# BBillot/SynthSR

Hardware: AMD Instinct MI355X
Metric: training volumes/sec (160^3 fp32, 5-level U-Net) (higher is better)
Workload: dtype f32; 1 GPU; configs[1]: brain_generator 160^3 batch=1 (training() defaults) + 5-level 3-D U-Net (24..384 features, Cin=2) fwd/bwd + Adam, fp32, random-init; global_batch=1, parallelism=dp1, conv_arithmetic=split

## Files before the change

include/synthsr_hip_tuning.h:

```cpp
#ifndef SYNTHSR_HIP_TUNING_H
#define SYNTHSR_HIP_TUNING_H
#ifdef __cplusplus
extern "C" {
#endif

int synthsr_split_tile_schedule(int kernel, int ntiles, int ny, int block_x, int block_yz, int out[4]);

int synthsr_set_deterministic(int on);
int synthsr_set_deterministic_workspace(void* planes, unsigned long long bytes);
unsigned long long synthsr_deterministic_workspace_demand(void);
int synthsr_deterministic_status(void);

#ifdef __cplusplus
}
#endif
#endif
```

synthsr_amd/_lib.py:

```python
import ctypes
import os
from ctypes import POINTER, Structure, c_char_p, c_double, c_float, c_int, c_int32, c_int64, c_uint32, c_uint64, c_void_p

_HERE = os.path.dirname(os.path.abspath(__file__))
LIB_PATH = os.environ.get('SYNTHSR_HIP_LIB') or os.path.join(_HERE, 'libsynthsr_hip.so')

_lib = None

I3 = c_int * 3
F12 = c_float * 12


class DeformParams(Structure):
    _fields_ = [('in_shape', c_int * 3), ('out_shape', c_int * 3), ('crop', c_int * 3), ('flip', c_int),
                ('has_field', c_int), ('has_affine', c_int), ('half_shape', c_int * 3), ('aff', c_float * 12),
                ('n_channels', c_int), ('lut_size', c_int), ('swap_lut_size', c_int), ('bias_on', c_int * 4),
                ('bias_shape', (c_int * 3) * 4), ('clip_hi', c_float), ('use_philox', c_int),
                ('philox_key', c_uint32 * 2), ('philox_offset', c_uint64), ('chan_first', c_int), ('n_channels_total', c_int),
                ('label_bytes', c_int)]


class ConvCtx(Structure):
    _fields_ = [('arithmetic', c_int), ('reserved0', c_int), ('workspace', c_void_p), ('workspace_bytes', c_uint64),
                ('reserved', c_int * 2)]


_P = c_void_p
_S = c_void_p
_C = POINTER(ConvCtx)

SIGNATURES = {
    'synthsr_abi_version': (c_int, []),
    'synthsr_build_arch': (c_char_p, []),
    'synthsr_resize_f32': (c_int, [_P, _P, c_int, POINTER(c_int), POINTER(c_int), c_int, _S]),
    'synthsr_svf_integrate': (c_int, [_P, _P, POINTER(c_int), c_int, _S]),
    'synthsr_affine_resample_linear': (c_int, [_P, _P, c_int, POINTER(c_int), POINTER(c_float), _S]),
    'synthsr_deform_gmm': (c_int, [_P, _P, _P, _P, _P, _P, _P, _P, _P, POINTER(DeformParams), _S]),
    'synthsr_mimic_acquisition': (c_int, [_P, _P, POINTER(c_int), POINTER(c_int), POINTER(c_float), POINTER(c_float),
                                          POINTER(c_float), c_int, c_int, c_int, _S]),
    'synthsr_deform_gmm_real': (c_int, [_P, _P, _P, _P, _P, _P, _P, _P, _P, _P, _P, _P, POINTER(DeformParams), _S]),
    'synthsr_minmax_init': (c_int, [_P, c_int, _S]),
    'synthsr_minmax_reduce': (c_int, [_P, c_int64, _P, _S]),
    'synthsr_normalise_gamma': (c_int, [_P, _P, c_int64, _P, c_float, _S]),
    'synthsr_blur3d': (c_int, [_P, _P, POINTER(c_int), _P, POINTER(c_int), c_int, c_int, c_int, c_float, _S]),
    'synthsr_normalise_blur2': (c_int, [_P, POINTER(c_int), _P, c_float, _P, _P, _P, _P, c_int, c_int, c_int, c_float, _S]),
    'synthsr_outer3': (c_int, [_P, _P, POINTER(c_int), c_int, c_int, _S]),
    'synthsr_copy_strided': (c_int, [_P, _P, c_int64, c_int, c_int, c_int, c_int, _S]),
    'synthsr_conv3d_pack': (c_int64, [_C, _P, _P, POINTER(c_int), c_int, c_int, c_int, _S]),
    'synthsr_conv3d_fwd': (c_int, [_C, _P, _P, _P, _P, POINTER(c_int), c_int, c_int, c_int, _S]),
    'synthsr_conv3d_fwd_stats': (c_int, [_C, _P, _P, _P, _P, POINTER(c_int), c_int, c_int, c_int, _P, _P, _S]),
    'synthsr_bn_stats_from_partials': (c_int, [_P, c_int, c_int64, c_int, _P, _S]),
    'synthsr_conv3d_fwd_add': (c_int, [_C, _P, _P, _P, _P, _P, POINTER(c_int), c_int, c_int, c_int, _S]),
    'synthsr_split_tile_schedule': (c_int, [c_int, c_int, c_int, c_int, c_int, POINTER(c_int)]),
    'synthsr_conv3d_wgrad_runs_split': (c_int, [_C, POINTER(c_int), c_int, c_int]),
    'synthsr_set_deterministic': (c_int, [c_int]),
    'synthsr_set_deterministic_workspace': (c_int, [_P, c_uint64]),
    'synthsr_deterministic_workspace_demand': (c_uint64, []),
    'synthsr_conv_workspace_bytes': (c_uint64, []),
    'synthsr_deterministic_status': (c_int, []),
    'synthsr_conv3d_plan': (c_int, [_C, POINTER(c_int), c_int, c_int, c_int, POINTER(c_int64)]),
    'synthsr_conv3d_pack_all': (c_int, [_P, _P, _P, c_int, _S]),
    'synthsr_conv3d_pack_ex': (c_int64, [_C, _P, _P, POINTER(c_int), c_int, c_int, c_int, c_int, c_int, c_int, _S]),
    'synthsr_conv3d_up_fwd': (c_int, [_C, _P, _P, _P, _P, _P, POINTER(c_int), c_int, c_int, c_int, _S]),
    'synthsr_conv3d_up_dgrad': (c_int, [_C, _P, _P, _P, POINTER(c_int), c_int, c_int, _S]),
    'synthsr_conv3d_up_wgrad': (c_int, [_C, _P, _P, _P, POINTER(c_int), c_int, c_int, _S]),
    'synthsr_conv3d_up_wgrad_runs_split': (c_int, [_C, POINTER(c_int), c_int, c_int]),
    'synthsr_conv3d_up_unpack': (c_int, [_P, _P, c_int, c_int, c_int, c_int, _S]),
    'synthsr_conv3d_wgrad_bias': (c_int, [_C, _P, _P, _P, _P, POINTER(c_int), c_int, c_int, c_int, c_int, _S]),
    'synthsr_conv3d_wgrad_ex': (c_int, [_C, _P, _P, _P, POINTER(c_int), c_int, c_int, c_int, c_int, _S]),
    'synthsr_conv3d_wgrad': (c_int, [_C, _P, _P, _P, POINTER(c_int), c_int, c_int, _S]),
    'synthsr_head_loss_fwd_ab': (c_int, [_P, POINTER(c_int), c_int, _P, _P, _P, c_float, _P, _P, _P, c_int, c_int, _P, _P, _P, _P, c_int, POINTER(c_int), _P, _S]),
    'synthsr_head_bwd_from_sums': (c_int, [_P, c_int, _P, _P, _P, _P, _P, _P, _S]),
    'synthsr_head_loss_fwd_bf16': (c_int, [_P, POINTER(c_int), c_int, _P, _P, _P, c_float, _P, _P, c_int, _P, c_int, POINTER(c_int), _P, _P, _P, _P, c_int, POINTER(c_int), _S]),
    'synthsr_conv3d_bf16_pack': (c_int64, [_P, _P, c_int, c_int, c_int, c_int, c_int, _S]),
    'synthsr_conv3d_bf16_pack_ex': (c_int64, [_P, _P, c_int, c_int, c_int, c_int, c_int, c_int, _S]),
    'synthsr_conv3d_bf16_pack_job': (c_int, [c_int, c_int, c_int, c_int, c_int, c_int, _P]),
    'synthsr_conv3d_bf16_wgrad_part': (c_int, [_P, _P, _P, _P, POINTER(c_int), c_int, c_int, c_int, c_int, _S]),
    'synthsr_conv3d_bf16_up_fwd': (c_int, [_P, _P, _P, POINTER(c_int), c_int, c_int, _S]),
    'synthsr_conv3d_bf16_up_dgrad': (c_int, [_P, _P, _P, POINTER(c_int), c_int, c_int, _P, c_int64, _S]),
    'synthsr_conv3d_bf16_up_wgrad': (c_int, [_P, _P, _P, POINTER(c_int), c_int, c_int, _S]),
    'synthsr_conv3d_bf16_pack_all': (c_int, [_P, _P, _P, c_int, _S]),
    'synthsr_conv3d_bf16_fwd': (c_int, [_P, _P, _P, _P, POINTER(c_int), c_int, c_int, c_int, _P, _P, _P, c_int64, _S]),
    'synthsr_conv3d_bf16_fwd_ex': (c_int, [_P, _P, _P, _P, POINTER(c_int), c_int, c_int, c_int, c_float, _P, _P, _P, c_int64, _S]),
    'synthsr_bf16_subsample_odd': (c_int, [_P, _P, _P, POINTER(c_int), c_int, c_float, _S]),
    'synthsr_bf16_zero_insert_odd': (c_int, [_P, _P, POINTER(c_int), c_int, _S]),
    'synthsr_conv3d_bf16_stats_scratch': (c_int64, [POINTER(c_int), c_int, c_int]),
    'synthsr_conv3d_bf16_wgrad': (c_int, [_P, _P, _P, _P, POINTER(c_int), c_int, c_int, c_int, c_int, _S]),
    'synthsr_f32_to_bf16_pad': (c_int, [_P, _P, c_int64, c_int, c_int, _S]),
    'synthsr_elu_bwd': (c_int, [_P, _P, _P, _P, _P, c_int64, c_int, _S]),
    'synthsr_scale_channels': (c_int, [_P, _P, c_int64, c_int, _P, c_int64, _S]),
    'synthsr_elu_bwd_drop': (c_int, [_P, _P, _P, _P, _P, c_int64, c_int, _P, _P, c_float, _P, _P, _P, _P, c_int64, _S]),
    'synthsr_bn_elu_bwd': (c_int, [_P, _P, _P, _P, _P, c_int64, c_int, _P, _P, c_float, _P, _S]),
    'synthsr_bn_stats': (c_int, [_P, c_int64, c_int, _P, _P, _S]),
    'synthsr_bn_apply': (c_int, [_P, _P, c_int64, c_int, _P, _P, _P, c_float, _S]),
    'synthsr_bn_maxpool': (c_int, [_P, _P, POINTER(c_int), c_int, _P, _P, _P, c_float, _S]),
    'synthsr_bn_maxpool_bwd': (c_int, [_P, _P, _P, POINTER(c_int), c_int, _P, _P, _P, c_float, _S]),
    'synthsr_bn_maxpool_bwd_ex': (c_int, [_P, _P, _P, POINTER(c_int), c_int, _P, _P, _P, c_float, _P, _S]),
    'synthsr_bn_pool_elu_bwd': (c_int, [_P, _P, _P, _P, _P, POINTER(c_int), c_int, _P, _P, _P, _P, c_float, _S]),
    'synthsr_act_bwd': (c_int, [_P, _P, _P, _P, _P, c_int64, c_int, c_int, _S]),
    'synthsr_bn_act_bwd': (c_int, [_P, _P, _P, _P, _P, c_int64, c_int, _P, _P, c_float, _P, c_int, _S]),
    'synthsr_bn_act_bwd_head': (c_int, [_P, _P, _P, _P, _P, c_int64, c_int, _P, _P, c_float, _P, c_int, _S]),
    'synthsr_act_bwd_drop': (c_int, [_P, _P, _P, _P, _P, c_int64, c_int, _P, _P, c_float, _P, _P, _P, _P, c_int64, c_int, _S]),
    'synthsr_bn_pool_act_bwd': (c_int, [_P, _P, _P, _P, _P, POINTER(c_int), c_int, _P, _P, _P, _P, c_float, c_int, _S]),
    'synthsr_bn_bwd_reduce': (c_int, [_P, _P, c_int64, c_int, _P, c_float, _P, _S]),
    'synthsr_bn_bwd_apply': (c_int, [_P, _P, _P, c_int64, c_int, _P, _P, c_float, _P, _S]),
    'synthsr_upsample_concat': (c_int, [_P, _P, _P, POINTER(c_int), c_int, c_int, _P, _P, _P, c_float, _S]),
    'synthsr_upsample_concat_bwd': (c_int, [_P, _P, _P, POINTER(c_int), c_int, c_int, _S]),
    'synthsr_head_l1_fwd': (c_int, [_P, c_int64, c_int, _P, _P, _P, c_float, _P, _P, _P, c_int, c_int, _P, _P, _P,
                                    _P, _S]),
    'synthsr_head_loss_fwd': (c_int, [_P, _P, c_int, _P, _P, _P, c_float, _P, _P, c_int, _P, c_int, _P, _P, _P, _P,
                                      _P, c_int, _P, _S]),
    'synthsr_head_bwd_multi': (c_int, [_P, _P, c_int64, c_int, c_int, _P, _P, _P, c_float, _P, _P, _P, _P, _S]),
    'synthsr_ssim_products': (c_int, [_P, _P, _P, _P, _P, _S]),
    'synthsr_ssim_filter': (c_int, [_P, _P, _P, c_int, c_int, c_int, _P, _S]),
    'synthsr_ssim_point': (c_int, [_P, c_int64, c_float, c_float, _P, _P, _S]),
    'synthsr_ssim_combine': (c_int, [_P, _P, _P, _P, _P, _P, _S]),
    'synthsr_conv3d_stride_unpack': (c_int, [_P, _P, c_int, c_int, _S]),
    'synthsr_bias_leaky_relu': (c_int, [_P, _P, _P, c_int64, c_int, c_float, _S]),
    'synthsr_colsum': (c_int, [_P, c_int64, c_int, _P, _S]),
    'synthsr_mul': (c_int, [_P, _P, _P, c_int64, _S]),
    'synthsr_lut_gather': (c_int, [_P, _P, c_int, _P, c_int64, _S]),
    'synthsr_leaky_relu': (c_int, [_P, _P, _P, c_int64, c_float, _S]),
    'synthsr_dense_fwd': (c_int, [_P, _P, _P, _P, c_int64, c_int, _S]),
    'synthsr_dense_bwd': (c_int, [_P, _P, _P, _P, _P, c_int64, c_int, _S]),
    'synthsr_axpby': (c_int, [_P, _P, _P, c_int64, c_float, c_float, _S]),
    'synthsr_sumsq': (c_int, [_P, c_int64, _P, _S]),
    'synthsr_bn_elu_bwd_head': (c_int, [_P, _P, _P, _P, _P, c_int64, c_int, _P, _P, c_float, _P, _S]),
    'synthsr_head_bwd_ex': (c_int, [_P, _P, c_int64, c_int, _P, _P, _P, c_float, _P, _P, _P, _P, _P, _S]),
    'synthsr_seg_head_fwd': (c_int, [_P, c_int64, c_int, _P, _P, _P, c_float, _P, _P, c_int, _P, _S]),
    'synthsr_seg_dice_sums': (c_int, [_P, _P, c_int64, c_int, _P, _P, c_int, _P, _S]),
    'synthsr_seg_dice_bwd': (c_int, [_P, _P, c_int64, c_int, c_int, _P, _P, _P, c_int, _P, c_float, _P, _S]),
    'synthsr_seg_head_dice_fwd': (c_int, [_P, c_int64, c_int, _P, _P, _P, c_float, _P, _P, c_int, _P, _P, c_int, _P, _P, _S]),
    'synthsr_seg_head_dice_bwd': (c_int, [_P, _P, _P, c_int, _P, c_int64, c_int, c_int, _P, _P, _P, c_float, _P, _P, c_float, _P,
                                          _P, _P, _S]),
    'synthsr_seg_head_argmax': (c_int, [_P, c_int64, c_int, _P, _P, _P, c_float, _P, _P, c_int, _P, _P, _S]),
    'synthsr_seg_head_tta_argmax': (c_int, [_P, POINTER(c_int), c_int, _P, _P, _P, c_float, _P, _P, c_int, _P, _P, _P, _P, _P,
                                            _S]),
    'synthsr_seg_label_counts': (c_int, [_P, _P, c_int64, _P, c_int, c_int, _P, _S]),
    'synthsr_head_bwd': (c_int, [_P, _P, c_int64, c_int, _P, _P, _P, c_float, _P, _P, _P, _P, _S]),
    'synthsr_adam_step': (c_int, [_P, _P, _P, _P, c_int64, c_float, c_float, c_float, c_float, c_float, _S]),
}

for _name in ('synthsr_elu_bwd', 'synthsr_bn_elu_bwd', 'synthsr_bn_elu_bwd_head', 'synthsr_elu_bwd_drop', 'synthsr_bn_pool_elu_bwd',
              'synthsr_act_bwd', 'synthsr_bn_act_bwd', 'synthsr_bn_act_bwd_head', 'synthsr_act_bwd_drop', 'synthsr_bn_pool_act_bwd',
              'synthsr_scale_channels', 'synthsr_bn_stats', 'synthsr_bn_apply', 'synthsr_bn_maxpool', 'synthsr_bn_maxpool_bwd',
              'synthsr_bn_maxpool_bwd_ex', 'synthsr_bn_bwd_reduce', 'synthsr_upsample_concat', 'synthsr_upsample_concat_bwd',
              'synthsr_head_loss_fwd_ab', 'synthsr_head_bwd_multi', 'synthsr_head_bwd_ex', 'synthsr_head_bwd'):
    SIGNATURES[_name + '_bf16'] = SIGNATURES[_name]


CONV_ARITHMETICS = ('fp32_mfma', 'split', 'split9')


class SynthSRHipError(RuntimeError):
    pass


def load():
    global _lib
    if _lib is not None:
        return _lib
    if not os.path.exists(LIB_PATH):
        raise SynthSRHipError('%s not found: build it with `python -m synthsr_amd.build` (hipcc, gfx950). '
                              'There is no CPU fallback.' % LIB_PATH)
    lib = ctypes.CDLL(LIB_PATH)
    for name, (res, args) in SIGNATURES.items():
        fn = getattr(lib, name)
        fn.restype = res
        fn.argtypes = args
    _lib = lib
    return lib


def check(rc, what='', planes=False):
    if rc == 0:
        return
    if rc == -1:
        raise ValueError('synthsr_hip: invalid argument / unsupported shape in %s' % what)
    if rc == -3 and planes:
        raise SynthSRHipError('synthsr_hip: %s needs more deterministic weight-gradient planes than the registered plane buffer '
                              'holds, even after registering a larger one (include/synthsr_hip_tuning.h: '
                              'synthsr_set_deterministic_workspace)' % what)
    if rc == -3:
        raise SynthSRHipError('synthsr_hip: %s needs scratch and the conv context carries no (or too small a) workspace '
                              '(include/synthsr_hip.h: synthsr_conv_ctx.workspace)' % what)
    raise SynthSRHipError('synthsr_hip: HIP launch error (%d) in %s' % (rc, what))


def i3(seq):
    return I3(*[int(s) for s in seq])


def ptr(t):
    if t is None:
        return None
    assert t.is_cuda and t.is_contiguous(), 'tensors handed to the HIP library must be contiguous device tensors'
    return c_void_p(t.data_ptr())


def stream():
    import torch
    return c_void_p(torch.cuda.current_stream().cuda_stream)
```

synthsr_amd/csrc/common.h:

```cpp
#pragma once
#include <hip/hip_runtime.h>
#include <stdint.h>
#include <type_traits>
#include "../../include/synthsr_hip.h"

#define SYN_CHECK_LAUNCH()                                 \
  do {                                                     \
    hipError_t e__ = hipGetLastError();                    \
    if (e__ != hipSuccess) return SYNTHSR_ELAUNCH;         \
  } while (0)

static inline int64_t syn_cdiv(int64_t a, int64_t b) { return (a + b - 1) / b; }

static inline int syn_grid(int64_t n, int block, int max_blocks = 256 * 16) {
  int64_t g = syn_cdiv(n, block);
  if (g > max_blocks) g = max_blocks;
  if (g < 1) g = 1;
  return (int)g;
}

#ifdef __HIPCC__
__device__ static inline void syn_block_range(int64_t n, int64_t& lo, int64_t& hi) {
  const int G = (int)gridDim.x, b = (int)blockIdx.x;
  const int pos = (G % 8 == 0) ? (b & 7) * (G >> 3) + (b >> 3) : b;
// ... 87 lines not shown
    }
    __syncthreads();
    if (tid < n) {
      double t = 0.0;
      for (int p = 0; p < P; ++p) t += s_col[p * n + tid];
      part[tid] = (float)t;
    }
  } else {
    for (int i = tid; i < n; i += nt) {
      double t = 0.0;
      for (int w = 0; w < nwg; ++w) t += (double)__builtin_nontemporal_load(d->scratch + (size_t)w * n + i);
      part[i] = (float)t;
    }
  }
  if (syn_tid0()) d->arrivals = 0;
  __syncthreads();
  return true;
}

__device__ __forceinline__ void syn_det_gather_end(int n) {
  SynDet* d = g_syn_det;
  if (d && (long long)syn_wg_count() * n > d->scratch_floats)
    syn_turn_end(&d->chain[SYN_DET_CHAINS - 1], syn_wg_linear(), syn_wg_count());
}

#include <atomic>
struct SynOncePerDevice {
  std::atomic<uint64_t> bits{0};
  bool needed() const {
    int dev = -1;
    if (hipGetDevice(&dev) != hipSuccess || dev < 0 || dev > 63) return true;
    return !(bits.load(std::memory_order_acquire) & (1ull << dev));
  }
  void done() {
    int dev = -1;
    if (hipGetDevice(&dev) == hipSuccess && dev >= 0 && dev <= 63) bits.fetch_or(1ull << dev, std::memory_order_release);
  }
  struct Guard {
    SynOncePerDevice* o;
    bool need;
    ~Guard() { if (need) o->done(); }
    explicit operator bool() const { return need; }
  };
  Guard first() { return Guard{this, needed()}; }
};
template <auto Kern>
void max_dyn_smem(size_t bytes) {
  static SynOncePerDevice done;
  if (auto once_ = done.first()) {
    (void)hipFuncSetAttribute(reinterpret_cast<const void*>(Kern), hipFuncAttributeMaxDynamicSharedMemorySize, (int)bytes);
  }
}
template <auto Kern, auto KernR, class... Args>
void launch_smem(bool relu, dim3 grid, dim3 block, size_t smem, hipStream_t st, Args... args) {
  if (relu) {
    max_dyn_smem<KernR>(smem);
    hipLaunchKernelGGL(KernR, grid, block, smem, st, args...);
  } else {
    max_dyn_smem<Kern>(smem);
    hipLaunchKernelGGL(Kern, grid, block, smem, st, args...);
  }
}

struct DetRun {
  float* planes = nullptr;
  float* dw = nullptr;
  float* dbias = nullptr;
  int64_t dw_elems = 0, stride = 0;
  int cout = 0, gx = 0;
};
extern "C" int syn_det_enabled();
extern "C" int syn_det_prepare(DetRun* d, float** dw, float** dbias, int64_t dw_elems, int cout, int gx, hipStream_t st);
extern "C" int syn_det_finish(const DetRun* d, hipStream_t st);

#define SYN_DET_SETTER(name)                                                                              \
  extern "C" __attribute__((visibility("hidden"))) int syn_det_set_##name(SynDet* p) {                   \
    return hipMemcpyToSymbol(HIP_SYMBOL(g_syn_det), &p, sizeof(p)) == hipSuccess ? 0 : 1;                 \
  }
#endif

__host__ __device__ static inline int syn_up_axis_taps(int p, int s, int t[2]) {
  if (p == 0) {
    if (s == 0) { t[0] = 0; return 1; }
    if (s == 1) { t[0] = 1; t[1] = 2; return 2; }
    return 0;
  }
  if (s == 1) { t[0] = 0; t[1] = 1; return 2; }
  if (s == 2) { t[0] = 2; return 1; }
  return 0;
}

__host__ __device__ static inline uint32_t syn_f2ord(float f) {
  union { float f; uint32_t u; } c;
  c.f = f;
  return (c.u & 0x80000000u) ? ~c.u : (c.u | 0x80000000u);
}
__host__ __device__ static inline float syn_ord2f(uint32_t u) {
  union { float f; uint32_t u; } c;
  c.u = (u & 0x80000000u) ? (u & 0x7fffffffu) : ~u;
  return c.f;
}

#ifdef __HIPCC__
__device__ __forceinline__ void syn_minmax_update(uint32_t* mm, float mn, float mx) {
  const uint32_t lo = syn_f2ord(mn), hi = syn_f2ord(mx);
  if (lo < __hip_atomic_load(&mm[0], __ATOMIC_RELAXED, __HIP_MEMORY_SCOPE_AGENT)) atomicMin(&mm[0], lo);
  if (hi > __hip_atomic_load(&mm[1], __ATOMIC_RELAXED, __HIP_MEMORY_SCOPE_AGENT)) atomicMax(&mm[1], hi);
}
#endif

#ifdef __HIPCC__
__device__ __forceinline__ uint32_t syn_pack_bf16x2(float lo, float hi) {
  typedef __bf16 syn_bf16x2 __attribute__((ext_vector_type(2)));
  const syn_bf16x2 v = {(__bf16)lo, (__bf16)hi};
  return __builtin_bit_cast(uint32_t, v);
}
__device__ __forceinline__ void syn_split3(float f0, float f1, uint32_t& p0, uint32_t& p1, uint32_t& p2) {
  p0 = syn_pack_bf16x2(f0, f1);
  float r0 = f0 - __uint_as_float(p0 << 16), r1 = f1 - __uint_as_float(p0 & 0xffff0000u);
  p1 = syn_pack_bf16x2(r0, r1);
  r0 -= __uint_as_float(p1 << 16);
  r1 -= __uint_as_float(p1 & 0xffff0000u);
  p2 = syn_pack_bf16x2(r0, r1);
}
#endif

#ifdef __HIPCC__
template <int I, int N, class F>
__device__ __forceinline__ void sfor(F&& f) {
  if constexpr (I < N) {
    f(std::integral_constant<int, I>{});
    sfor<I + 1, N>(f);
  }
}

__device__ __forceinline__ float elu_f(float v) {
  const float e = __builtin_amdgcn_exp2f(v * 1.44269504088896341f) - 1.f;
  const float p = v * fmaf(v, fmaf(v, fmaf(v, fmaf(v, 1.f / 120.f, 1.f / 24.f), 1.f / 6.f), 0.5f), 1.f);
  const float n = v > -0.125f ? p : e;
  return v > 0.f ? v : n;
}
__device__ __forceinline__ float elu_dy(float y) { return y > 0.f ? 1.f : y + 1.f; }
template <bool RELU>
__device__ __forceinline__ float act_f(float v) {
  if constexpr (RELU) return fmaxf(v, 0.f);
  else return elu_f(v);
}
template <bool RELU>
__device__ __forceinline__ float act_dy(float y) {
  if constexpr (RELU) return y > 0.f ? 1.f : 0.f;
  else return elu_dy(y);
}

constexpr int TZ = 4, TY = 4, TX = 16, HZ = TZ + 2, HY = TY + 2, HX = TX + 2, HVOX = HZ * HY * HX;
constexpr int SLAB_Z = 4;
__device__ __forceinline__ void tile_decode(int p, int tiles0, int tiles1, int tiles2, int& z0, int& y0, int& x0) {
  const int t12 = tiles1 * tiles2;
  const int s = p / (SLAB_Z * t12), r = p - s * SLAB_Z * t12;
  const int sz = min(SLAB_Z, tiles0 - s * SLAB_Z);
  const int t1 = r / (sz * tiles2), rr = r - t1 * sz * tiles2;
  const int zz = rr / tiles2, t2 = rr - zz * tiles2;
  z0 = (s * SLAB_Z + zz) * TZ;
  y0 = t1 * TY;
  x0 = t2 * TX;
}
#endif
static inline int syn_tile_grid_x(int slots, int ntiles) {
  int gx = slots / 8 * 8;
  if (gx < 8) gx = 8;
  while (gx > 8 && gx - 8 >= ntiles) gx -= 8;
  if (ntiles < 8) gx = ntiles;
  return gx;
}

__host__ __device__ inline bool syn_split_replanned(int vox_tiles, int co_tiles, int mt) {
  if (mt != 2 || co_tiles <= 3 || (co_tiles % 3) != 0 || (co_tiles % 2) != 0) return false;
  const long long u3 = (long long)vox_tiles * (co_tiles / 3);
  return u3 > 512 && u3 < 768;
}
__host__ __device__ inline int syn_split_plan_mt(int vox_tiles, int co_tiles, bool replan) {
  const int mt = co_tiles <= 3 ? co_tiles : ((co_tiles % 3) == 0 ? 3 : ((co_tiles % 2) == 0 ? 2 : 1));
  if (replan && mt == 3 && syn_split_replanned(vox_tiles, co_tiles, 2)) return 2;
  return mt;
}

__host__ __device__ constexpr int syn_split_tap(int slot) {
  const int p = slot >> 1, h = slot & 1;
  if (p < 9) return p * 3 + 2 * h;
  const int i = 2 * (p - 9) + h;
  return i < 9 ? i * 3 + 1 : -1;
}
__host__ __device__ constexpr int syn_split_tap8(int slot) {
  const int p = slot >> 1, h = slot & 1;
  return 4 * (p & 1) + 2 * h + (p >> 1);
}
__host__ __device__ constexpr int syn_split_voxel(int m) { return m < 4 ? 2 * m : (m >= 12 ? 2 * m - 16 : 2 * m - 7); }

__device__ static inline float syn_wave_sum(float v) {
#pragma unroll
  for (int o = 32; o > 0; o >>= 1) v += __shfl_xor(v, o, 64);
  return v;
}
__device__ static inline float syn_wave_min(float v) {
#pragma unroll
  for (int o = 32; o > 0; o >>= 1) v = fminf(v, __shfl_xor(v, o, 64));
  return v;
}
__device__ static inline float syn_wave_max(float v) {
#pragma unroll
  for (int o = 32; o > 0; o >>= 1) v = fmaxf(v, __shfl_xor(v, o, 64));
  return v;
}
```

synthsr_amd/csrc/conv3d.hip:

```cpp
#include "common.h"
#include <algorithm>
#include <cstddef>

SYN_DET_SETTER(conv3d)

namespace {

typedef float f32x4 __attribute__((ext_vector_type(4)));

constexpr int MAX_NT = 6;

__host__ __device__ inline int cdiv(int a, int b) { return (a + b - 1) / b; }

inline int ck_for(int Cin) { return (Cin % 24 == 0) ? 24 : 8; }
inline int ck_for_fwd(int Cin) { return (Cin % 24 == 0) ? 24 : ((Cin % 32 == 0) ? 32 : 8); }

typedef unsigned int u32x4 __attribute__((ext_vector_type(4)));
typedef unsigned int u32x2 __attribute__((ext_vector_type(2)));
__device__ __forceinline__ float4 ld4(const float* p) { return *reinterpret_cast<const float4*>(p); }

__device__ __forceinline__ int up_axis_taps(int p, int s, int t[2]) {
  if (p == 0) {
    if (s == 0) { t[0] = 0; return 1; }
    if (s == 1) { t[0] = 1; t[1] = 2; return 2; }
// ... 2462 lines not shown
      if (i < NJ - 1 || tid + 256 * i < PLANE4) {
#pragma unroll
        for (int hz = 0; hz < FH0; ++hz)
          *reinterpret_cast<float4*>(&lds[ldsa[i] + hz * (FH1 * FH2 * CKP)]) = stg[hz * NJ + i];
      }
    }
    __syncthreads();
    const bool has_next = t + G < ntiles;
    if (has_next) load_halo(t + G);
    int nz0 = z0, ny0 = y0, nx0 = x0;
    if (has_next) tile_origin(t + G, nz0, ny0, nx0);
    for (int z = 0; z < FT0; ++z) {
      float ar[8][3];
#pragma unroll
      for (int o = 0; o < 8; ++o)
#pragma unroll
        for (int r = 0; r < 3; ++r) ar[o][r] = an[o][r];
      if (z + 1 < FT0) {
        load_dz(z0, y0, x0, z + 1, an);
      } else if (has_next) {
        load_dz(nz0, ny0, nx0, 0, an);
      }
      int rb[NQ];
#pragma unroll
      for (int q = 0; q < NQ; ++q) rb[q] = rowoff[q] + z * (FH1 * FH2 * CKP);
      float xq[2][NQ];
#pragma unroll
      for (int q = 0; q < NQ; ++q) xq[0][q] = lds[rb[q]];
      sfor<0, 64>([&](auto S) {
        constexpr int sv = decltype(S)::value, o = sv / 8, k = sv % 8;
        constexpr int sn = sv + 1 < 64 ? sv + 1 : sv, on = sn / 8, kn = sn % 8;
        constexpr int nbase = ((on >> 1) * FH2 + 8 * (on & 1) + kn) * CKP;
#pragma unroll
        for (int q = 0; q < NQ; ++q) xq[(sv + 1) & 1][q] = lds[rb[q] + nbase];
        __builtin_amdgcn_sched_barrier(0);
        sfor<0, 6>([&](auto GI) {
          constexpr int g = decltype(GI)::value, GG = k * 6 + g;
#pragma unroll
          for (int q = 0; q < NQ; ++q)
            acc[q][g] = __builtin_amdgcn_mfma_f32_4x4x1f32(ar[o][GG / 16], xq[sv & 1][q], acc[q][g], 4, GG % 16, 0);
        });
        __builtin_amdgcn_sched_barrier(0);
      });
    }
    z0 = nz0;
    y0 = ny0;
    x0 = nx0;
  }
  dwc += (size_t)blockIdx.x * det_stride;
  for (int w = 0; w < 4; ++w) {
    __syncthreads();
    if (wave == w) {
#pragma unroll
      for (int q = 0; q < NQ; ++q) {
        const int blk = 16 * q + (lane >> 2);
        float* d = lds + (blk * 4 + (lane & 3)) * Cout;
#pragma unroll
        for (int g = 0; g < 6; ++g)
          *reinterpret_cast<float4*>(d + 4 * g) = make_float4(acc[q][g][0], acc[q][g][1], acc[q][g][2], acc[q][g][3]);
      }
    }
    __syncthreads();
    const int wp = (blockIdx.y & 1) * 4 + w, wz = (wp >> 2) & 1, wy = (wp >> 1) & 1, wx = wp & 1;
    float* dst = dwc + (size_t)wp * dwstride;
    for (int e = tid; e < 8 * CK * Cout; e += 256) {
      const int ti = e / (CK * Cout), r = e - ti * (CK * Cout);
      const int tap = ((wz + ((ti >> 2) & 1)) * 3 + (wy + ((ti >> 1) & 1))) * 3 + (wx + (ti & 1));
      atomicAdd(dst + ((size_t)tap * Cin + cc * CK) * Cout + r, lds[e]);
    }
  }
}

__global__ __launch_bounds__(256) void colsum_kernel(const float* __restrict__ x, int64_t n, int C,
                                                     float* __restrict__ out) {
  __shared__ float part[256];
  const int rows = C <= 256 ? 256 / C : 1;
  int* turn = nullptr;
  for (int c0 = 0; c0 < C; c0 += 256) {
    const int width = min(256, C - c0);
    const int r = threadIdx.x / width, c = threadIdx.x - r * width;
    float acc = 0.f;
    if (r < rows)
      for (int64_t v = (int64_t)blockIdx.x * rows + r; v < n; v += (int64_t)gridDim.x * rows) acc += x[v * C + c0 + c];
    part[threadIdx.x] = acc;
    __syncthreads();
    if (c0 == 0) turn = syn_turn_begin(0, blockIdx.x);
    if (threadIdx.x < width) {
      float t = 0.f;
      for (int k = 0; k < rows; ++k) t += part[k * width + threadIdx.x];
      atomicAdd(out + c0 + threadIdx.x, t);
    }
    __syncthreads();
  }
  syn_turn_end(turn, blockIdx.x, gridDim.x);
}

constexpr int SYN_MAX_DEVICES = 64;
struct SynDeviceState {
  int det = 0;
  SynDet* det_state = nullptr;
  float* det_planes = nullptr;
  size_t det_planes_floats = 0;
  unsigned long long det_demand_bytes = 0;
};
static SynDeviceState g_dev[SYN_MAX_DEVICES];
static SynDeviceState g_dev_invalid;
static SynDeviceState& dev_state() {
  int d = -1;
  if (hipGetDevice(&d) != hipSuccess || d < 0 || d >= SYN_MAX_DEVICES) return g_dev_invalid;
  return g_dev[d];
}
static inline int det_on() { return dev_state().det; }

constexpr int PLAN_KS_TARGET = 1024;
constexpr int PLAN_SPLIT_MIN_WGS = 200;

struct ConvCfg {
  int arith;
  int split;
  int nprod;
  void* ws;
  size_t ws_bytes;
};
static thread_local ConvCfg t_cfg = {1, 1, 6, nullptr, 0};
static inline const ConvCfg& cfg() { return t_cfg; }
struct CtxScope {
  ConvCfg prev;
  bool ok;
  explicit CtxScope(const synthsr_conv_ctx* ctx) : prev(t_cfg), ok(true) {
    const int a = ctx ? ctx->arithmetic : SYNTHSR_ARITH_SPLIT;
    if (a < 0 || a > 2 || (ctx && (ctx->reserved0 || ctx->reserved[0] || ctx->reserved[1] || (ctx->workspace_bytes && !ctx->workspace)))) {
      ok = false;
      return;
    }
    t_cfg = ConvCfg{a, a ? 1 : 0, a == 2 ? 9 : 6, ctx ? ctx->workspace : nullptr, ctx ? (size_t)ctx->workspace_bytes : 0};
  }
  ~CtxScope() { t_cfg = prev; }
};
constexpr size_t SYN_WORKSPACE_BOUND = (size_t)16 << 20;
static float* ctx_scratch(size_t bytes) {
  static_assert((size_t)2048 * 1536 * sizeof(float) <= SYN_WORKSPACE_BOUND, "first-layer weight-gradient partials");
  return (bytes <= SYN_WORKSPACE_BOUND && bytes <= cfg().ws_bytes) ? static_cast<float*>(cfg().ws) : nullptr;
}

extern "C" int syn_split_wgrad(const float* in, const float* dout, float* dw, float* dbias, const int s[3], int cin_total,
                               int ci_off, int Cin, int Cout, int nprod, hipStream_t st);
extern "C" int syn_split_upwgrad(const float* lo, const float* dout, float* dwc, const int s[3], int Cin, int Cout, int nprod,
                                 hipStream_t st);
extern "C" int syn_split_upfwd(const float* lo, const float* wp, const float* bias, const float* addend, float* out,
                               const int s[3], int Cin, int Cout, int mt, int act, int nprod, hipStream_t st);
extern "C" int syn_split_fwd_halves(const int s[3], int Cin, int nchunks, int stacked, int nprod);
extern "C" int syn_split_fwd(const float* in, const float* wp, const float* bias, const float* addend, float* out,
                             const int s[3], int Cin, int Cout, int mt, int nchunks, int act, float* stats, float* partial,
                             int upm, int stacked, int nprod, hipStream_t st);

inline bool wgrad_takes_split(const int s[3], int Cin, int Cout) {
  const int64_t vox = (int64_t)s[0] * s[1] * s[2];
  return cfg().split && (Cin % 8) == 0 && (Cout % 24) == 0 && vox * Cin * 4 < (1ll << 31) && vox * Cout * 4 < (1ll << 31);
}

inline bool up_wgrad_takes_split(const int s[3], int Cl, int Cout) {
  const int64_t vox = (int64_t)s[0] * s[1] * s[2];
  return cfg().split && cfg().nprod == 6 && (Cl % 16) == 0 && (Cout % 24) == 0 && vox * Cl * 4 < (1ll << 31) &&
         8 * vox * Cout * 4 < (1ll << 31);
}

struct FwdPlan {
  int nt, mt, ksplit, nchunks, ncc, ck, persist, p4, c2, brick, wn, wm, split, stacked;
  int pack_nt() const { return stacked ? -400 : split == 3 ? -300 - mt : (split == 2 ? -200 - mt : (split ? -100 - mt : (c2 ? -c2 : (p4 ? 0 : nt)))); }
  int64_t count() const {
    if (stacked) return (int64_t)ncc * 7 * 5 * 64 * 4;
    if (split) return (int64_t)3 * nchunks * ncc * (split >= 2 ? 2 : 7) * mt * 64 * 4;
    if (c2) return (int64_t)((27 * c2 * 6 + 15) / 16) * 64;
    if (p4) return (int64_t)ncc * 27 * 9 * 64;
    return (int64_t)nchunks * ncc * 27 * (ck / 8) * nt * 128;
  }
};

inline FwdPlan plan_fwd(const int s[3], int Cin, int Cout, int kind = 1) {
  const bool plain = kind == 1;
  FwdPlan p;
  p.split = 0;
  p.stacked = 0;
  if (cfg().split && (Cin % 8) == 0 && (Cout % 8) == 0) {
    const int64_t vox = (int64_t)s[0] * s[1] * s[2];
    const int ntiles = cdiv(Cout, 16);
    const int mt = syn_split_plan_mt(cdiv(s[0], 4) * cdiv(s[1], 4) * cdiv(s[2], 16), ntiles, kind != 2);
    const int nchunks = cdiv(ntiles, mt);
    const int64_t wgs = (int64_t)cdiv(s[0], 4) * cdiv(s[1], 4) * cdiv(s[2], 16) * nchunks;
    if (wgs >= PLAN_SPLIT_MIN_WGS && (kind == 0 ? 8 : 1) * vox * Cin * 4 < (1ll << 31) && (kind == 2 ? 8 : 1) * vox * Cout * 4 < (1ll << 31) &&
        (kind != 2 || nchunks == 1)) {
      p.split = plain ? 1 : (kind == 0 ? 2 : 3);
      p.ck = 8;
      p.ncc = Cin / 8;
      p.mt = mt;
      p.nt = mt;
      p.nchunks = nchunks;
      p.ksplit = 1;
      p.stacked = (plain && Cout == 24 && cfg().arith == 1) ? 1 : 0;
      p.persist = p.p4 = p.c2 = p.brick = 0;
      p.wn = p.wm = 1;
      return p;
    }
  }
  p.ck = ck_for_fwd(Cin);
  p.ncc = cdiv(Cin, p.ck);
  const int ntiles = cdiv(Cout, 16);
  auto wgs = [&](int mt, int nt) { return (int64_t)cdiv(s[0], FT0) * cdiv(s[1], mt) * cdiv(s[2], FT2) * cdiv(ntiles, nt); };
  p.mt = 4;
  int max_nt = MAX_NT;
  if (wgs(4, std::min(MAX_NT, ntiles)) < 768 || p.ck == 32) {
    p.mt = 2;
    max_nt = 3;
  }
  p.nchunks = cdiv(ntiles, max_nt);
  p.nt = cdiv(ntiles, p.nchunks);
  p.ksplit = 1;
  const bool lt2g = (int64_t)s[0] * s[1] * s[2] * Cin * 4 < (1ll << 31);
  p.persist = (p.mt == 4 && p.ck == 24 && p.nt <= 3 && (Cout % 4) == 0 && lt2g) ? 1 : 0;
  p.p4 = (p.persist && (kind == 1 || kind == 2) && Cout == 24 && (Cin % 24) == 0) ? 1 : 0;
  p.c2 = (plain && Cout == 24 && Cin <= 2 && lt2g) ? Cin : 0;
  p.brick = 0;
  p.wn = 1;
  p.wm = 1;
  if (p.ck == 24 && p.mt == 2 && lt2g && (Cout % 16) == 0 && (s[0] % 4) == 0 && (s[1] % 4) == 0 && (s[2] % 4) == 0 &&
      (s[2] % 16) != 0) {
    p.brick = 1;
    p.nt = (ntiles % 3 == 0) ? 3 : ((ntiles % 2 == 0) ? 2 : 1);
    p.nchunks = ntiles / p.nt;
    p.wn = (p.nchunks % 4 == 0) ? 4 : ((p.nchunks % 2 == 0) ? 2 : 1);
    p.wm = (p.wn <= 2 && (s[1] % 8) == 0) ? 2 : 1;
    if (p.wn == 1) {
      p.brick = 0;
      p.wm = 1;
      p.nchunks = cdiv(ntiles, max_nt);
      p.nt = cdiv(ntiles, p.nchunks);
    }
  }
  if (p.brick) {
    const int64_t w = (int64_t)(s[0] / 4) * (s[1] / (4 * p.wm)) * (s[2] / 4) * (p.nchunks / p.wn);
    p.ksplit = 1;
    if (w < 400 && p.ncc >= 2 && plain) {
      int ks = (int)cdiv(PLAN_KS_TARGET, (int)w);
      if (ks > p.ncc) ks = p.ncc;
      if (ks > 16) ks = 16;
      if (ks >= 2 && !det_on()) p.ksplit = ks;
    }
    return p;
  }
  const int64_t w = wgs(p.mt, p.nt);
  if (w < 512 && p.ncc >= 4 && plain) {
    int ks = (int)cdiv(PLAN_KS_TARGET, (int)w);
    if (ks > p.ncc / 2) ks = p.ncc / 2;
    if (ks > 8) ks = 8;
    if (ks >= 2 && !det_on()) p.ksplit = ks;
  }
  return p;
}

inline int parity_split(int64_t workgroups, const float* bias, int act, const ConvExt& ext) {
  if (det_on() || bias != nullptr || act != 0 || ext.addend != nullptr) return 1;
  int ps = 1;
  while (ps < 8 && workgroups * ps < 400) ps *= 2;
  return ps;
}

inline bool launch_act(int& act) {
  const bool relu = act >= 3;
  if (relu) act -= 2;
  return relu;
}

inline int splitk_begin(float* out, int64_t nout, int act, const ConvExt& ext, hipStream_t st) {
  if (ext.mode != 0) return SYNTHSR_EINVAL;
  if (act != 2 && ext.addend && ext.addend != out) return SYNTHSR_EINVAL;
  if ((act == 2 || !ext.addend) && hipMemsetAsync(out, 0, (size_t)nout * sizeof(float), st) != hipSuccess) return SYNTHSR_ELAUNCH;
  return SYNTHSR_OK;
}
inline int splitk_end(float* out, const float* bias, int64_t nout, int Cout, int act, bool relu, const ConvExt& ext,
                      hipStream_t st) {
  if (bias == nullptr && act == 0) return SYNTHSR_OK;
  hipLaunchKernelGGL((relu ? bias_act_kernel<true> : bias_act_kernel<false>), dim3(syn_grid(nout, 256)), dim3(256), 0, st, out,
                     bias, nout, Cout, act, act == 2 ? ext.addend : nullptr);
  return hipGetLastError() == hipSuccess ? SYNTHSR_OK : SYNTHSR_ELAUNCH;
}

template <int CK, int NT, int MT, bool KS>
int launch_fwd(const float* in, const float* wp, const float* bias, float* out, const int s[3], int Cin, int Cout,
               const FwdPlan& pl, int act, hipStream_t st, const ConvExt& ext) {
  const bool relu = launch_act(act);
  const int tiles0 = cdiv(s[0], FT0), tiles1 = cdiv(s[1], MT), tiles2 = cdiv(s[2], FT2);
  const size_t smem = (size_t)FH0 * (MT + 2) * FH2 * (CK + 4) * sizeof(float);
  const int64_t nout = (int64_t)s[0] * s[1] * s[2] * Cout;
  enum { GENERIC, LEAN27, LEAN8 } kern = GENERIC;
  if constexpr (CK == 24 && NT <= 3) {
    const int64_t in_bytes = (int64_t)s[0] * s[1] * s[2] * (ext.mode == 2 ? 8 : 1) * Cin * 4;
    const int64_t w_bytes = pl.count() * 4 * (ext.mode ? 8 : 1);
    if (in_bytes < (1ll << 31) && w_bytes < (1ll << 31)) kern = ext.mode == 0 ? LEAN27 : LEAN8;
  }
  if (KS) {
    if (const int rc = splitk_begin(out, nout, act, ext, st)) return rc;
  }
  int gz = KS ? pl.ksplit : (ext.mode == 1 ? 8 : 1);
  if (!KS && kern == LEAN8 && ext.mode == 2) {
    gz = parity_split((int64_t)tiles0 * tiles1 * tiles2 * pl.nchunks, bias, act, ext);
    if (gz > 1 && hipMemsetAsync(out, 0, (size_t)nout * sizeof(float), st) != hipSuccess) return SYNTHSR_ELAUNCH;
  }
// ... 517 lines not shown
      return syn_det_finish(&det, st);
    }
  }
  if constexpr (NTAPS == 27) {
    if (Cin <= 2 && Cout == 24 && (int64_t)shape[0] * shape[1] * shape[2] * Cout * 4 < (1ll << 31))
      return launch_wgrad_c2(in, dout, dw, ext.dbias, shape, Cin, st, ext);
    if (wgrad_takes_split(shape, Cin, Cout)) {
      const int rc = syn_split_wgrad(in, dout, dw, ext.dbias, shape, ext.cin_total, ext.ci_off, Cin, Cout, cfg().nprod, st);
      if (rc != SYNTHSR_EINVAL) return rc;
    }
  }
  if constexpr (NTAPS == 27) {
    const int64_t vox = (int64_t)shape[0] * shape[1] * shape[2];
    if (Cout == 24 && (Cin % 24) == 0 && vox * Cin * 4 < (1ll << 31) && vox * Cout * 4 < (1ll << 31)) {
      const int tiles0 = cdiv(shape[0], FT0), tiles1 = cdiv(shape[1], 4), tiles2 = cdiv(shape[2], FT2);
      const int ntiles = tiles0 * tiles1 * tiles2, ncc = Cin / 24;
      const size_t smem = (size_t)FH0 * 6 * FH2 * 28 * sizeof(float);
      max_dyn_smem<conv3d_wgrad_p4_kernel>(smem);
      int gx = std::max(8, ((512 / ncc) / 8) * 8);
      while (gx > 8 && gx > ntiles) gx -= 8;
      DetRun det;
      float* dbias = ext.dbias;
      if (const int rc_ = syn_det_prepare(&det, &dw, &dbias, (int64_t)27 * ext.cin_total * Cout, Cout, gx, st)) return rc_;
      hipLaunchKernelGGL(conv3d_wgrad_p4_kernel, dim3(gx, ncc), dim3(256), smem, st, in, dout, dw, shape[0], shape[1],
                         shape[2], Cin, tiles1, tiles2, ntiles, ext.cin_total, ext.ci_off, dbias, det.stride);
      if (hipGetLastError() != hipSuccess) return SYNTHSR_ELAUNCH;
      return syn_det_finish(&det, st);
    }
  }
  const int CK = ck_for(Cin);
  const int nt_all = cdiv(Cout, 16);
  const int nco = cdiv(nt_all, 3);
  const int NT = cdiv(nt_all, nco);
  if (CK == 24) {
    if (NT == 1) return launch_wgrad<24, 1, 1, NTAPS>(in, dout, dw, shape, Cin, Cout, st, ext);
    if (NT == 2) return launch_wgrad<24, 2, 1, NTAPS>(in, dout, dw, shape, Cin, Cout, st, ext);
    if constexpr (NTAPS == 27) return launch_wgrad<24, 3, 2, 27>(in, dout, dw, shape, Cin, Cout, st, ext);
    return launch_wgrad<24, 3, 1, NTAPS>(in, dout, dw, shape, Cin, Cout, st, ext);
  }
  if (NT == 1) return launch_wgrad<8, 1, 1, NTAPS>(in, dout, dw, shape, Cin, Cout, st, ext);
  if (NT == 2) return launch_wgrad<8, 2, 1, NTAPS>(in, dout, dw, shape, Cin, Cout, st, ext);
  return launch_wgrad<8, 3, 1, NTAPS>(in, dout, dw, shape, Cin, Cout, st, ext);
}

}

extern "C" {

int64_t synthsr_conv3d_pack_ex(const synthsr_conv_ctx* ctx, const float* w, float* packed, const int shape[3], int Cin_total,
                               int ci_off, int Cin, int Cout, int mode, int up, synthsr_stream_t stream) {
  const CtxScope scope(ctx);
  if (!scope.ok) return SYNTHSR_EINVAL;
  if (!shape || Cin < 1 || Cout < 1 || ci_off < 0 || ci_off + Cin > Cin_total || (mode != 0 && mode != 1) ||
      shape[0] < 1 || shape[1] < 1 || shape[2] < 1 || up < 0 || up > 2)
    return SYNTHSR_EINVAL;
  const int CinE = mode ? Cout : Cin, CoutE = mode ? Cin : Cout;
  const int kind = !up ? 1 : ((up == 1) == (mode == 0) ? 2 : 0);
  const FwdPlan pl = plan_fwd(shape, CinE, CoutE, kind);
  const int64_t per = pl.count();
  if (per >= (1ll << 31)) return SYNTHSR_EINVAL;
  const int64_t total = per * (up ? 8 : 1);
  if (!packed) return total;
  if (!w) return SYNTHSR_EINVAL;
  for (int p = 0; p < (up ? 8 : 1); ++p) {
    hipLaunchKernelGGL(pack_kernel, dim3(syn_grid(per, 256)), dim3(256), 0, (hipStream_t)stream, w, packed + p * per,
                       Cin_total, ci_off, Cin, Cout, mode, pl.ck, pl.ncc, pl.pack_nt(), pl.nchunks,
                       up ? p + (up == 2 ? 8 : 0) : -1, per);
    if (hipGetLastError() != hipSuccess) return SYNTHSR_ELAUNCH;
  }
  return total;
}

int64_t synthsr_conv3d_pack(const synthsr_conv_ctx* ctx, const float* w, float* packed, const int shape[3], int Cin, int Cout,
                            int mode, synthsr_stream_t stream) {
  return synthsr_conv3d_pack_ex(ctx, w, packed, shape, Cin, 0, Cin, Cout, mode, 0, stream);
}

int synthsr_conv3d_plan(const synthsr_conv_ctx* ctx, const int shape[3], int CinE, int CoutE, int plain, int64_t out[8]) {
  const CtxScope scope(ctx);
  if (!scope.ok) return SYNTHSR_EINVAL;
  if (!shape || !out || CinE < 1 || CoutE < 1 || shape[0] < 1 || shape[1] < 1 || shape[2] < 1) return SYNTHSR_EINVAL;
  const FwdPlan pl = plan_fwd(shape, CinE, CoutE, plain);
  out[0] = pl.ck;
  out[1] = pl.ncc;
  out[2] = pl.pack_nt();
  out[3] = pl.nchunks;
  out[4] = pl.mt;
  out[5] = (pl.split == 1 && syn_split_fwd_halves(shape, CinE, pl.nchunks, pl.stacked, cfg().nprod)) ? 2 : pl.ksplit;
  out[6] = 0;
  out[7] = pl.count();
  return SYNTHSR_OK;
}

int synthsr_conv3d_wgrad_runs_split(const synthsr_conv_ctx* ctx, const int shape[3], int Cin, int Cout) {
  const CtxScope scope(ctx);
  if (!scope.ok) return SYNTHSR_EINVAL;
  if (!shape || Cin < 1 || Cout < 1 || shape[0] < 1 || shape[1] < 1 || shape[2] < 1) return SYNTHSR_EINVAL;
  return (Cin > 2 || Cout != 24) && wgrad_takes_split(shape, Cin, Cout) ? 1 : 0;
}

int synthsr_conv3d_up_wgrad_runs_split(const synthsr_conv_ctx* ctx, const int lo_shape[3], int Cl, int Cout) {
  const CtxScope scope(ctx);
  if (!scope.ok) return SYNTHSR_EINVAL;
  if (!lo_shape || Cl < 1 || Cout < 1 || lo_shape[0] < 1 || lo_shape[1] < 1 || lo_shape[2] < 1) return SYNTHSR_EINVAL;
  return up_wgrad_takes_split(lo_shape, Cl, Cout) ? 1 : 0;
}

int synthsr_conv3d_pack_all(const float* params, float* packed, const int64_t* jobs_dev, int njobs,
                            synthsr_stream_t stream) {
  if (!params || !packed || !jobs_dev || njobs < 1) return SYNTHSR_EINVAL;
  hipLaunchKernelGGL(pack_all_kernel, dim3(256, njobs), dim3(256), 0, (hipStream_t)stream, params, packed, jobs_dev);
  return hipGetLastError() == hipSuccess ? SYNTHSR_OK : SYNTHSR_ELAUNCH;
}

__global__ void stride_unpack_kernel(const float* __restrict__ dwc, float* __restrict__ dw, int Ci, int Co, int64_t total) {
  for (int64_t idx = blockIdx.x * (int64_t)blockDim.x + threadIdx.x; idx < total; idx += (int64_t)gridDim.x * blockDim.x) {
    const int co = (int)(idx % Co);
    const int ci = (int)((idx / Co) % Ci);
    const int t = (int)(idx / ((int64_t)Co * Ci));
    const int tz = t / 9, ty = (t / 3) % 3, tx = t % 3;
    const int p = ((tz & 1) << 2) | ((ty & 1) << 1) | (tx & 1);
    const int slot = ((1 - (tz >> 1)) * 3 + (1 - (ty >> 1))) * 3 + (1 - (tx >> 1));
    dw[idx] += dwc[(((int64_t)p * 27 + slot) * Co + co) * Ci + ci];
  }
}

int synthsr_conv3d_stride_unpack(const float* dwc, float* dw, int Ci, int Co, synthsr_stream_t stream) {
  if (!dwc || !dw || Ci < 1 || Co < 1) return SYNTHSR_EINVAL;
  const int64_t total = (int64_t)27 * Ci * Co;
  hipLaunchKernelGGL(stride_unpack_kernel, dim3(syn_grid(total, 256)), dim3(256), 0, (hipStream_t)stream, dwc, dw, Ci, Co,
                     total);
  return hipGetLastError() == hipSuccess ? SYNTHSR_OK : SYNTHSR_ELAUNCH;
}

int synthsr_conv3d_up_unpack(float* dwc, float* dw, int Cin_total, int ci_off, int Cl, int Cout, synthsr_stream_t stream) {
  if (!dwc || !dw || Cl < 1 || Cout < 1 || ci_off < 0 || ci_off + Cl > Cin_total) return SYNTHSR_EINVAL;
  const int64_t total = (int64_t)27 * Cl * Cout;
  hipLaunchKernelGGL(up_unpack_kernel, dim3(syn_grid(total, 256)), dim3(256), 0, (hipStream_t)stream, dwc, dw, Cin_total,
                     ci_off, Cl, Cout, total);
  if (hipGetLastError() != hipSuccess) return SYNTHSR_ELAUNCH;
  const int64_t total64 = (int64_t)64 * Cl * Cout;
  hipLaunchKernelGGL(up_clear_kernel, dim3(syn_grid(total64, 256)), dim3(256), 0, (hipStream_t)stream, dwc, Cl, Cout, total64);
  return hipGetLastError() == hipSuccess ? SYNTHSR_OK : SYNTHSR_ELAUNCH;
}

int synthsr_conv3d_fwd(const synthsr_conv_ctx* ctx, const float* in, const float* wpacked, const float* bias, float* out,
                       const int shape[3], int Cin, int Cout, int act, synthsr_stream_t stream) {
  const CtxScope scope(ctx);
  if (!scope.ok) return SYNTHSR_EINVAL;
  if (!conv_args_ok(in, wpacked, out, shape, Cin, Cout) || (act != 0 && act != 1 && act != 3)) return SYNTHSR_EINVAL;
  const FwdPlan pl = plan_fwd(shape, Cin, Cout);
  if (pl.split)
    return syn_split_fwd(in, wpacked, bias, nullptr, out, shape, Cin, Cout, pl.mt, pl.nchunks, act, nullptr, nullptr, 0,
                         pl.stacked, cfg().nprod, (hipStream_t)stream);
  return dispatch_fwd_ck(pl, in, wpacked, bias, out, shape, Cin, Cout, act, stream, ConvExt{0, nullptr, 0});
}

int synthsr_conv3d_fwd_add(const synthsr_conv_ctx* ctx, const float* in, const float* wpacked, const float* bias,
                           const float* addend, float* out, const int shape[3], int Cin, int Cout, int act,
                           synthsr_stream_t stream) {
  const CtxScope scope(ctx);
  if (!scope.ok) return SYNTHSR_EINVAL;
  if (!conv_args_ok(in, wpacked, out, shape, Cin, Cout) || act < 0 || act > 4 ||
      ((act == 2 || act == 4) && (!addend || addend == out)))
    return SYNTHSR_EINVAL;
  const FwdPlan pl = plan_fwd(shape, Cin, Cout);
  if (pl.split)
    return syn_split_fwd(in, wpacked, bias, addend, out, shape, Cin, Cout, pl.mt, pl.nchunks, act, nullptr, nullptr, 0,
                         pl.stacked, cfg().nprod, (hipStream_t)stream);
  return dispatch_fwd_ck(pl, in, wpacked, bias, out, shape, Cin, Cout, act, stream, ConvExt{0, addend, 0});
}

int synthsr_conv3d_fwd_stats(const synthsr_conv_ctx* ctx, const float* in, const float* wpacked, const float* bias, float* out,
                             const int shape[3], int Cin, int Cout, int act, float* stats, double* ws, synthsr_stream_t stream) {
  const CtxScope scope(ctx);
  if (!scope.ok) return SYNTHSR_EINVAL;
  if (!conv_args_ok(in, wpacked, out, shape, Cin, Cout) || !stats || !ws || (act != 0 && act != 1 && act != 3))
    return SYNTHSR_EINVAL;
  const int64_t nvox = (int64_t)shape[0] * shape[1] * shape[2];
  const FwdPlan pl = plan_fwd(shape, Cin, Cout);
  if (pl.split) {
    float* partial = ctx_scratch((size_t)512 * 2 * Cout * sizeof(float));
    if (!partial) return SYNTHSR_EWORKSPACE;
    return syn_split_fwd(in, wpacked, bias, nullptr, out, shape, Cin, Cout, pl.mt, pl.nchunks, act, stats, partial, 0,
                         pl.stacked, cfg().nprod, (hipStream_t)stream);
  }
  if (pl.p4 && nvox * Cin * 4 < (1ll << 31))
    return launch_fwd_p4(in, wpacked, bias, out, shape, Cin, pl, act, (hipStream_t)stream, nullptr, stats);
  const int rc = synthsr_conv3d_fwd(ctx, in, wpacked, bias, out, shape, Cin, Cout, act, stream);
  if (rc != SYNTHSR_OK) return rc;
  return synthsr_bn_stats(out, nvox, Cout, stats, ws, stream);
}

int synthsr_conv3d_up_fwd(const synthsr_conv_ctx* ctx, const float* lo, const float* wpacked8, const float* bias,
                          const float* addend, float* out, const int lo_shape[3], int Cl, int Cout, int act,
                          synthsr_stream_t stream) {
  const CtxScope scope(ctx);
  if (!scope.ok) return SYNTHSR_EINVAL;
  if (!conv_args_ok(lo, wpacked8, out, lo_shape, Cl, Cout) || (act != 0 && act != 1 && act != 3)) return SYNTHSR_EINVAL;
  const FwdPlan pl = plan_fwd(lo_shape, Cl, Cout, 2);
  if (pl.split)
    return syn_split_upfwd(lo, wpacked8, bias, addend, out, lo_shape, Cl, Cout, pl.mt, act, cfg().nprod, (hipStream_t)stream);
  return dispatch_fwd_ck(pl, lo, wpacked8, bias, out, lo_shape, Cl, Cout, act, stream, ConvExt{1, addend, pl.count()});
}

int synthsr_conv3d_up_dgrad(const synthsr_conv_ctx* ctx, const float* dout, const float* wpacked8, float* dlo,
                            const int lo_shape[3], int Cl, int Cout, synthsr_stream_t stream) {
  const CtxScope scope(ctx);
  if (!scope.ok) return SYNTHSR_EINVAL;
  if (!conv_args_ok(dout, wpacked8, dlo, lo_shape, Cl, Cout)) return SYNTHSR_EINVAL;
  const FwdPlan pl = plan_fwd(lo_shape, Cout, Cl, 0);
  if (pl.split)
    return syn_split_fwd(dout, wpacked8, nullptr, nullptr, dlo, lo_shape, Cout, Cl, pl.mt, pl.nchunks, 0, nullptr, nullptr, 2, 0,
                         cfg().nprod, (hipStream_t)stream);
  return dispatch_fwd_ck(pl, dout, wpacked8, nullptr, dlo, lo_shape, Cout, Cl, 0, stream, ConvExt{2, nullptr, pl.count()});
}


extern "C" __attribute__((visibility("hidden"))) int syn_det_enabled() { return det_on(); }
extern "C" __attribute__((visibility("hidden"))) int syn_det_prepare(DetRun* d, float** dw, float** dbias, int64_t dw_elems,
                                                                      int cout, int gx, hipStream_t st) {
  return det_prepare_impl(d, dw, dbias, dw_elems, cout, gx, st);
}
extern "C" __attribute__((visibility("hidden"))) int syn_det_finish(const DetRun* d, hipStream_t st) {
  return det_finish_impl(d, st);
}
extern "C" int syn_det_set_pointwise(SynDet*);
extern "C" int syn_det_set_critic(SynDet*);
extern "C" int syn_det_set_ssim(SynDet*);
extern "C" int syn_det_set_conv_bf16(SynDet*);
constexpr long long DET_SCRATCH_FLOATS = 16ll << 20;

int synthsr_set_deterministic(int on) {
  if (hipDeviceSynchronize() != hipSuccess) return SYNTHSR_ELAUNCH;
  int cur = -1;
  if (hipGetDevice(&cur) != hipSuccess || cur < 0 || cur >= SYN_MAX_DEVICES) return SYNTHSR_EINVAL;
  SynDeviceState& ds = g_dev[cur];
  if (on && !ds.det_state) {
    SynDet* state = nullptr;
    float* scratch = nullptr;
    if (hipMalloc(reinterpret_cast<void**>(&state), sizeof(SynDet)) != hipSuccess) return SYNTHSR_ELAUNCH;
    bool ok = hipMalloc(reinterpret_cast<void**>(&scratch), DET_SCRATCH_FLOATS * sizeof(float)) == hipSuccess;
    if (ok) {
      SynDet* h = new SynDet();
      h->scratch_floats = DET_SCRATCH_FLOATS;
      h->scratch = scratch;
      ok = hipMemcpy(state, h, sizeof(SynDet), hipMemcpyHostToDevice) == hipSuccess;
      delete h;
    }
    if (!ok) {
      if (scratch) (void)hipFree(scratch);
      (void)hipFree(state);
      return SYNTHSR_ELAUNCH;
    }
    ds.det_state = state;
  }
  if (ds.det_state) {
    if (hipMemset(ds.det_state, 0, offsetof(SynDet, scratch_floats)) != hipSuccess) return SYNTHSR_ELAUNCH;
    if (hipMemset(reinterpret_cast<char*>(ds.det_state) + offsetof(SynDet, chain), 0, sizeof(int) * SYN_DET_CHAINS) != hipSuccess)
      return SYNTHSR_ELAUNCH;
  }
  SynDet* p = on ? ds.det_state : nullptr;
  ds.det = on ? 1 : 0;
  if (syn_det_set_conv3d(p) || syn_det_set_pointwise(p) || syn_det_set_critic(p) || syn_det_set_ssim(p) ||
      syn_det_set_conv_bf16(p))
    return SYNTHSR_ELAUNCH;
  return hipDeviceSynchronize() == hipSuccess ? SYNTHSR_OK : SYNTHSR_ELAUNCH;
}

int synthsr_set_deterministic_workspace(void* planes, unsigned long long bytes) {
  if (hipDeviceSynchronize() != hipSuccess) return SYNTHSR_ELAUNCH;
  int d = -1;
  if (hipGetDevice(&d) != hipSuccess || d < 0 || d >= SYN_MAX_DEVICES || (bytes && !planes)) return SYNTHSR_EINVAL;
  SynDeviceState& ds = g_dev[d];
  ds.det_planes = static_cast<float*>(planes);
  ds.det_planes_floats = planes ? (size_t)(bytes / sizeof(float)) : 0;
  return SYNTHSR_OK;
}

unsigned long long synthsr_deterministic_workspace_demand(void) { return dev_state().det_demand_bytes; }

unsigned long long synthsr_conv_workspace_bytes(void) { return (unsigned long long)SYN_WORKSPACE_BOUND; }

int synthsr_deterministic_status(void) {
  const SynDeviceState& ds = dev_state();
  if (!ds.det) return 0;
  int v[2] = {0, 0};
  if (hipMemcpy(v, ds.det_state, sizeof(v), hipMemcpyDeviceToHost) != hipSuccess) return -1;
  return v[1] ? 2 : 1;
}

int synthsr_conv3d_wgrad_bias(const synthsr_conv_ctx* ctx, const float* in, const float* dout, float* dw, float* dbias,
                              const int shape[3], int Cin_total, int ci_off, int Cin, int Cout, synthsr_stream_t stream) {
  const CtxScope scope(ctx);
  if (!scope.ok) return SYNTHSR_EINVAL;
  if (!conv_args_ok(in, dout, dw, shape, Cin, Cout) || ci_off < 0 || ci_off + Cin > Cin_total) return SYNTHSR_EINVAL;
  const WgExt ext{0, Cin_total, ci_off, 0, dbias};
  return dispatch_wgrad<27>(in, dout, dw, shape, Cin, Cout, (hipStream_t)stream, ext);
}

int synthsr_conv3d_wgrad_ex(const synthsr_conv_ctx* ctx, const float* in, const float* dout, float* dw, const int shape[3],
                            int Cin_total, int ci_off, int Cin, int Cout, synthsr_stream_t stream) {
  return synthsr_conv3d_wgrad_bias(ctx, in, dout, dw, nullptr, shape, Cin_total, ci_off, Cin, Cout, stream);
}

int synthsr_conv3d_wgrad(const synthsr_conv_ctx* ctx, const float* in, const float* dout, float* dw, const int shape[3], int Cin,
                         int Cout, synthsr_stream_t stream) {
  return synthsr_conv3d_wgrad_ex(ctx, in, dout, dw, shape, Cin, 0, Cin, Cout, stream);
}

int synthsr_conv3d_up_wgrad(const synthsr_conv_ctx* ctx, const float* lo, const float* dout, float* dwc, const int lo_shape[3],
                            int Cl, int Cout, synthsr_stream_t stream) {
  const CtxScope scope(ctx);
  if (!scope.ok) return SYNTHSR_EINVAL;
  if (!conv_args_ok(lo, dout, dwc, lo_shape, Cl, Cout)) return SYNTHSR_EINVAL;
  const WgExt ext{1, Cl, 0, (int64_t)27 * Cl * Cout, nullptr};
  return dispatch_wgrad<8>(lo, dout, dwc, lo_shape, Cl, Cout, (hipStream_t)stream, ext);
}

}
```

synthsr_amd/csrc/conv_split.hip:

```cpp
#include "common.h"
#include <algorithm>
#include <type_traits>
#include <utility>

#ifdef SYN_SPLIT_TIMING
static __device__ long long* g_tm = nullptr;
extern "C" int synthsr_split_timing_buffer(long long* p) {
  return hipMemcpyToSymbol(HIP_SYMBOL(g_tm), &p, sizeof(p)) == hipSuccess ? 0 : 1;
}
#define TM(i) do { if (g_tm && (blockIdx.x == 0 || blockIdx.x == 300) && blockIdx.y == 0 && tid == 0 && tix < 120) g_tm[((blockIdx.x ? 1 : 0) * 120 + tix) * 8 + (i)] = clock64(); } while (0)
#define T2(k) do { if (g_tm && threadIdx.x == 0 && ((blockIdx.x == 7 && blockIdx.y == 0) || (blockIdx.x == 20 && blockIdx.y == 1)) && n2 < 400) { g_tm[(blockIdx.y * 400 + n2) * 2] = (k); g_tm[(blockIdx.y * 400 + n2) * 2 + 1] = clock64(); ++n2; } } while (0)
#else
#define TM(i)
#define T2(k)
#endif
#ifdef SYN_SPLIT_TIMING
#define T3(i) do { if (g_tm && lane == 0 && blockIdx.x == 7 && blockIdx.y == 0 && n3 < 48) g_tm[1600 + ((tid >> 6) * 48 + n3) * 2 + (i)] = clock64(); } while (0)
#else
#define T3(i)
#endif


namespace {

// ... 231 lines not shown
      xload(0, 0);
      sfor<0, NSTEP>([&](auto S) {
        constexpr int s = decltype(S)::value;
        constexpr bool last = s + 1 == NSTEP;
        const u32x4* wn = last ? wf_next : wf;
        constexpr int sn = last ? 0 : s + 1;
        if constexpr (NPROD == 9) {
          __builtin_amdgcn_sched_barrier(0);
          mma(I0{}, I2{});
          mma(I0{}, I1{});
          mma(I0{}, I0{});
          __builtin_amdgcn_sched_barrier(0);
          wload(wn, sn, 0);
          __builtin_amdgcn_sched_barrier(0);
          mma(I1{}, I2{});
          mma(I1{}, I1{});
          mma(I1{}, I0{});
          __builtin_amdgcn_sched_barrier(0);
          wload(wn, sn, 1);
          __builtin_amdgcn_sched_barrier(0);
          mma(I2{}, I2{});
          mma(I2{}, I1{});
          mma(I2{}, I0{});
          __builtin_amdgcn_sched_barrier(0);
          wload(wn, sn, 2);
          if constexpr (!last) {
            xload(sn, 2);
            xload(sn, 1);
            xload(sn, 0);
          }
          return;
        }
        __builtin_amdgcn_sched_barrier(0);
        mma(I0{}, I2{});
        __builtin_amdgcn_sched_barrier(0);
        if constexpr (!last) xload(sn, 2);
        __builtin_amdgcn_sched_barrier(0);
        mma(I0{}, I1{});
        __builtin_amdgcn_sched_barrier(0);
        mma(I0{}, I0{});
        __builtin_amdgcn_sched_barrier(0);
        wload(wn, sn, 0);
        __builtin_amdgcn_sched_barrier(0);
        mma(I1{}, I0{});
        __builtin_amdgcn_sched_barrier(0);
        mma(I1{}, I1{});
        __builtin_amdgcn_sched_barrier(0);
        wload(wn, sn, 1);
        if constexpr (!last) xload(sn, 1);
        __builtin_amdgcn_sched_barrier(0);
        mma(I2{}, I0{});
        __builtin_amdgcn_sched_barrier(0);
        wload(wn, sn, 2);
        if constexpr (!last) xload(sn, 0);
      });
      __builtin_amdgcn_sched_barrier(0);
      TM(3);
#ifdef SYN_SPLIT_TIMING
      asm volatile("s_waitcnt vmcnt(0)" ::: "memory");
      TM(6);
#endif
      if (more) store_halo(buf ^ 1);
      TM(4);
      buf ^= 1;
    }
    int z0, y0, x0;
    tile_decode(t, tiles0, a.tiles1, a.tiles2, z0, y0, x0);
    const int gz = z0 + wave, gx = x0 + xv;
    const bool zx_ok = gz < D0 && gx < D2;
    const uint32_t row0 = (uint32_t)((gz * D1 + y0) * D2 + gx) * (uint32_t)(Cout * 4);
    const uint32_t ystep = (uint32_t)(D2 * Cout * 4);
    auto epi = [&](auto ACTC, auto ADDC) {
      constexpr int ACT = decltype(ACTC)::value;
      constexpr bool ADD = decltype(ADDC)::value;
#pragma unroll
      for (int mt = 0; mt < MT; ++mt) {
        const int co = (chunk * MT + mt) * 16 + 4 * g;
        f32x4 bias = {0.f, 0.f, 0.f, 0.f};
        if (a.bias && co < Cout) bias = *reinterpret_cast<const f32x4*>(a.bias + co);
#pragma unroll
        for (int y = 0; y < TY; ++y) {
          const bool vok = zx_ok && (y0 + y) < D1;
          const uint32_t off = (vok && co < Cout) ? row0 + y * ystep + (uint32_t)(co * 4) : OOB;
          f32x4 v;
#pragma unroll
          for (int i = 0; i < 4; ++i) v[i] = acc[y][mt][i] + bias[i];
          if constexpr (ADD || ACT == 2) {
            const f32x4 b = __builtin_bit_cast(f32x4, __builtin_amdgcn_raw_buffer_load_b128(radd, (int)off, 0, 0));
#pragma unroll
            for (int i = 0; i < 4; ++i) v[i] = ACT == 2 ? v[i] * act_dy<RELU>(b[i]) : v[i] + b[i];
          }
          if constexpr (ACT == 1) {
#pragma unroll
            for (int i = 0; i < 4; ++i) v[i] = act_f<RELU>(v[i]);
          }
          __builtin_amdgcn_raw_buffer_store_b128(__builtin_bit_cast(u32x4, v), rout, (int)off, 0, 0);
          if constexpr (ST) {
            const float w = off != OOB ? 1.f : 0.f;
#pragma unroll
            for (int i = 0; i < 4; ++i) {
              const float r = w * v[i];
              s1[mt][i] += r;
              s2[mt][i] += r * r;
            }
          }
        }
      }
    };
    using T_ = std::true_type;
    using F_ = std::false_type;
    if constexpr (ST) {
      if (a.act == 1) epi(std::integral_constant<int, 1>{}, F_{});
      else epi(std::integral_constant<int, 0>{}, F_{});
    } else {
      if (a.act == 2) epi(std::integral_constant<int, 2>{}, F_{});
      else if (a.addend) {
        if (a.act == 1) epi(std::integral_constant<int, 1>{}, T_{});
        else epi(std::integral_constant<int, 0>{}, T_{});
      } else if (a.act == 1) epi(std::integral_constant<int, 1>{}, F_{});
      else epi(std::integral_constant<int, 0>{}, F_{});
    }
    TM(5);
  }
  if constexpr (ST) {
    __syncthreads();
    float* red = reinterpret_cast<float*>(lds);
#pragma unroll
    for (int mt = 0; mt < MT; ++mt)
#pragma unroll
      for (int i = 0; i < 4; ++i) {
        float x1 = s1[mt][i], x2 = s2[mt][i];
#pragma unroll
        for (int o = 8; o > 0; o >>= 1) {
          x1 += __shfl_xor(x1, o, 64);
          x2 += __shfl_xor(x2, o, 64);
        }
        if (m == 0) {
          red[(wave * 2 + 0) * (MT * 16) + mt * 16 + 4 * g + i] = x1;
          red[(wave * 2 + 1) * (MT * 16) + mt * 16 + 4 * g + i] = x2;
        }
      }
    __syncthreads();
    float* dst = a.stats_partial + (int64_t)blockIdx.x * (2 * Cout);
    for (int e = tid; e < MT * 16; e += 256) {
      const int c = chunk * MT * 16 + e;
      if (c < Cout) {
        dst[c] = red[e] + red[2 * MT * 16 + e] + red[4 * MT * 16 + e] + red[6 * MT * 16 + e];
        dst[Cout + c] = red[MT * 16 + e] + red[3 * MT * 16 + e] + red[5 * MT * 16 + e] + red[7 * MT * 16 + e];
      }
    }
  }
}

constexpr int PLANE2 = 6 * 256 * 8;
constexpr int BUF2 = 3 * PLANE2;
static_assert(PLANE2 >= PLANE, "padded plane holds the halo image");
constexpr int STK_TILES = 5;

constexpr int epi_base(int epi) { return epi == 5 ? 1 : (epi == 6 ? 2 : (epi == 7 ? 4 : epi)); }

template <int MT, bool ST, int EPI0, bool STK, int KS = 1>
__global__ __launch_bounds__(256 * KS, KS == 1 ? 2 : 1) void conv3d_split_fwd2_kernel(const SplitFwdArgs a) {
  static_assert(KS == 1 || (KS == 2 && !STK), "split-K halves: the plain layout");
  constexpr int NSTEP = NSTEP27;
  constexpr int TYE = TY / KS;
  constexpr int NITEM = TYE * MT;
  constexpr int NWT = STK ? STK_TILES : MT;
  constexpr int EPI = epi_base(EPI0);
  constexpr bool RELU = EPI0 >= 5;
  static_assert(!ST || EPI <= 1, "statistics belong to plain forward convs");
  static_assert(!STK || MT == 2, "the stacked layout is the 24-channel one (two output tiles)");
  extern __shared__ __attribute__((aligned(16))) unsigned char lds[];
  const int half = KS == 1 ? 0 : __builtin_amdgcn_readfirstlane((int)threadIdx.x >> 8);
  const int tid = threadIdx.x & 255, lane = tid & 63, wave = tid >> 6;
  unsigned char* const ldsh = lds + half * (2 * BUF2);
  const int m = lane & 15, g = lane >> 4;
  const int chunk = blockIdx.y, nchunks = gridDim.y;
  const TileWalk walk = tile_walk(a.ntiles);
  const int tiles0 = a.ntiles / (a.tiles1 * a.tiles2);
  const int D0 = a.D0, D1 = a.D1, D2 = a.D2, Cin = a.Cin, Cout = a.Cout, ncc = a.ncc;

  int koff[NSTEP];
#pragma unroll
  for (int s = 0; s < NSTEP; ++s) {
    int tap = syn_split_tap(4 * s + g);
    if (tap < 0) tap = syn_split_tap((4 * s + g) ^ 1);
    koff[s] = ((tap / 9 * HY + (tap / 3) % 3) * HX + tap % 3) * 16;
  }
  const int xv = syn_split_voxel(m);
  const int lbase = (wave * HY * HX + xv) * 16;

  constexpr int NP = HVOX * 2, NL = 6;
  static_assert(NL * 256 >= NP, "six staging pieces per thread cover the halo image");
  int prel[NL];
  uint32_t pmask[NL];
#pragma unroll
  for (int i = 0; i < NL; ++i) {
    const int j = tid + 256 * i;
    const int v = j >> 1, h = j & 1;
    const int hz = v / (HY * HX), r = v - hz * (HY * HX), hy = r / HX, hx = r - hy * HX;
    prel[i] = ((hz * D1 + hy) * D2 + hx) * Cin * 4 + h * 16;
    pmask[i] = j < NP ? ((1u << hz) | (1u << (6 + hy)) | (1u << (12 + hx))) : 0xFFFFFFFFu;
  }
  const int plds0 = (tid >> 1) * 16 + (tid & 1) * 8;
  const __amdgpu_buffer_rsrc_t rin =
      __builtin_amdgcn_make_buffer_rsrc(const_cast<float*>(a.in), 0, (int)((int64_t)D0 * D1 * D2 * Cin * 4), 0x00020000);
  f32x4 stg[NL];
  uint32_t hbad = 0;
  int hbase = 0;
  int hw_tile = -1, hw_base0 = 0;
  uint32_t hw_bad = 0;
  auto halo_where = [&](int t, int cc, bool none) {
    if (t != hw_tile) {
      int z0, y0, x0;
      tile_decode(t, tiles0, a.tiles1, a.tiles2, z0, y0, x0);
      uint32_t bad = 0x80000000u;
      bad |= syn_oob_bits(z0 - 1, HZ, D0) | (syn_oob_bits(y0 - 1, HY, D1) << 6) | (syn_oob_bits(x0 - 1, HX, D2) << 12);
      hw_bad = bad;
      hw_base0 = (((z0 - 1) * D1 + (y0 - 1)) * D2 + (x0 - 1)) * Cin * 4;
      hw_tile = t;
    }
    hbad = none ? 0xFFFFFFFFu : hw_bad;
    hbase = hw_base0 + cc * 32;
  };
  auto load_pieces = [&](auto I0_, auto I1_) {
    constexpr int i0 = decltype(I0_)::value, i1 = decltype(I1_)::value;
#pragma unroll
    for (int i = i0; i < i1; ++i) {
      const uint32_t vo = (pmask[i] & hbad) ? OOB : (uint32_t)(prel[i] + hbase);
      stg[i] = __builtin_bit_cast(f32x4, __builtin_amdgcn_raw_buffer_load_b128(rin, (int)vo, 0, 0));
    }
  };
  using P0 = std::integral_constant<int, 0>;
  using P4 = std::integral_constant<int, 4>;
  using P6 = std::integral_constant<int, 6>;
  typedef unsigned int u32x2 __attribute__((ext_vector_type(2)));
  uint32_t cp[6];
  auto conv_a = [&](int i) { syn_split3(stg[i][0], stg[i][1], cp[0], cp[1], cp[2]); };
  auto conv_b = [&](int i) { syn_split3(stg[i][2], stg[i][3], cp[3], cp[4], cp[5]); };
  auto conv_c = [&](int i, unsigned char* dst) {
    *reinterpret_cast<u32x2*>(dst + plds0 + i * 2048) = (u32x2){cp[0], cp[3]};
    *reinterpret_cast<u32x2*>(dst + PLANE2 + plds0 + i * 2048) = (u32x2){cp[1], cp[4]};
    *reinterpret_cast<u32x2*>(dst + 2 * PLANE2 + plds0 + i * 2048) = (u32x2){cp[2], cp[5]};
  };

  const int64_t piece_stride = (int64_t)nchunks * ncc * NSTEP * MT * 64;
  const u32x4* __restrict__ wbase = a.wp + (STK ? 0 : (int64_t)chunk * ncc * NSTEP * MT * 64) + lane;
  constexpr int WCHUNK = NSTEP * NWT * 64;

  float s1[ST ? MT : 1][4], s2[ST ? MT : 1][4];
#pragma unroll
  for (int mt = 0; mt < (ST ? MT : 1); ++mt)
#pragma unroll
    for (int i = 0; i < 4; ++i) s1[mt][i] = s2[mt][i] = 0.f;

  const int64_t out_bytes = (int64_t)D0 * D1 * D2 * Cout * 4;
  const __amdgpu_buffer_rsrc_t rout = __builtin_amdgcn_make_buffer_rsrc(a.out, 0, (int)out_bytes, 0x00020000);
  const __amdgpu_buffer_rsrc_t radd = __builtin_amdgcn_make_buffer_rsrc(
      const_cast<float*>(a.addend ? a.addend : a.out), 0, (int)out_bytes, 0x00020000);
  const uint32_t ystep = (uint32_t)(D2 * Cout * 4);

  float* lbias = reinterpret_cast<float*>(lds + KS * 2 * BUF2);
  if ((int)threadIdx.x < MT * 16) {
    const int co = chunk * MT * 16 + tid;
    lbias[tid] = (a.bias && co < Cout) ? a.bias[co] : 0.f;
  }

  u32x4 wa[STK ? 1 : 3][STK ? STK_TILES : MT], xb[3][TY];
  auto wload = [&](const u32x4* wf, int s, int q) {
    if constexpr (!STK) {
#pragma unroll
      for (int mt = 0; mt < MT; ++mt) wa[q][mt] = wf[q * piece_stride + (s * MT + mt) * 64];
    }
  };
  auto wload_t = [&](const u32x4* wf, int s, int tl) {
    if constexpr (STK) wa[0][tl] = wf[(s * STK_TILES + tl) * 64];
  };
  using I0 = std::integral_constant<int, 0>;
  using I1 = std::integral_constant<int, 1>;
  using I2 = std::integral_constant<int, 2>;
  using I3 = std::integral_constant<int, 3>;
  using I4 = std::integral_constant<int, 4>;

  f32x4 acc[TY][NWT];
  constexpr int EA = EPI >= 2 ? 3 : 1, ENB = EA + 1;
  f32x4 ev, eb[ENB];
  uint32_t eoff[ENB];
  auto epi0 = [&](int j, uint32_t row0, uint32_t yok) {
    const int mt = j / TYE, y = j % TYE;
    const int co = (chunk * MT + mt) * 16 + 4 * g;
    eoff[j % ENB] = (((yok >> y) & 1u) && co < Cout) ? row0 + (uint32_t)y * ystep + (uint32_t)(co * 4) : OOB;
    if constexpr (EPI >= 2)
      eb[j % ENB] = __builtin_bit_cast(f32x4, __builtin_amdgcn_raw_buffer_load_b128(radd, (int)eoff[j % ENB], 0, 0));
  };
  auto epi1 = [&](int j) {
    const int mt = j / TYE, y = j % TYE;
    const f32x4 bj = *reinterpret_cast<const f32x4*>(lbias + mt * 16 + 4 * g);
    f32x4 v;
    if constexpr (STK) {
      if (mt == 0) {
#pragma unroll
        for (int i = 0; i < 4; ++i) v[i] = (acc[y][0][i] + acc[y][1][i]) + acc[y][2][i];
      } else {
#pragma unroll
        for (int i = 0; i < 4; ++i) v[i] = (acc[y][3][i] + __shfl_down(acc[y][3][i], 32, 64)) + acc[y][4][i];
      }
    } else {
      v = acc[y][mt];
    }
#pragma unroll
    for (int i = 0; i < 4; ++i) v[i] += bj[i];
    if constexpr (EPI == 2) {
#pragma unroll
      for (int i = 0; i < 4; ++i) v[i] *= act_dy<RELU>(eb[j % ENB][i]);
    }
    if constexpr (EPI == 3 || EPI == 4) {
#pragma unroll
      for (int i = 0; i < 4; ++i) v[i] += eb[j % ENB][i];
    }
    if constexpr (EPI == 1 || EPI == 4) {
#pragma unroll
      for (int i = 0; i < 4; ++i) v[i] = act_f<RELU>(v[i]);
    }
    ev = v;
  };
  auto epi2 = [&](int j) {
    __builtin_amdgcn_raw_buffer_store_b128(__builtin_bit_cast(u32x4, ev), rout, (int)eoff[j % ENB], 0, 0);
    if constexpr (ST) {
      const int mt = j / TYE;
      const float w = eoff[j % ENB] != OOB ? 1.f : 0.f;
#pragma unroll
      for (int i = 0; i < 4; ++i) {
        const float r = w * ev[i];
        s1[mt][i] += r;
        s2[mt][i] += r * r;
      }
    }
  };

  int buf = 0;
  int n2 = 0;
  (void)n2;
  T2(0);
  if (walk.pos < walk.end) {
    halo_where(walk.pos, half, false);
    load_pieces(P0{}, P6{});
#pragma unroll
    for (int i = 0; i < NL; ++i) {
      conv_a(i);
      conv_b(i);
      conv_c(i, ldsh);
    }
    if constexpr (STK) {
#pragma unroll
      for (int tl = 0; tl < STK_TILES; ++tl) wload_t(wbase, 0, tl);
    } else {
      wload(wbase + (int64_t)half * WCHUNK, 0, 0);
      wload(wbase + (int64_t)half * WCHUNK, 0, 1);
      wload(wbase + (int64_t)half * WCHUNK, 0, 2);
    }
  }
  T2(1);
  for (int t = walk.pos; t < walk.end; t += walk.stride) {
#pragma unroll
    for (int y = 0; y < TY; ++y)
#pragma unroll
      for (int tl = 0; tl < NWT; ++tl) acc[y][tl] = (f32x4){0.f, 0.f, 0.f, 0.f};
    for (int cc = half; cc < ncc; cc += KS) {
      T2(2);
      __syncthreads();
      T2(3);
      const bool last_cc = cc + KS >= ncc;
      const bool more = !last_cc || t + walk.stride < walk.end;
      halo_where(last_cc ? (more ? t + walk.stride : t) : t, last_cc ? half : cc + KS, !more);
      load_pieces(P0{}, P4{});
      const u32x4* wf = wbase + (int64_t)cc * WCHUNK;
      const u32x4* wf_next = wbase + (int64_t)(last_cc ? half : cc + KS) * WCHUNK;
      const unsigned char* img = ldsh + buf * BUF2 + lbase;
      unsigned char* nimg = ldsh + (buf ^ 1) * BUF2;
      auto xload = [&](int s, int q) {
#pragma unroll
        for (int y = 0; y < TY; ++y) xb[q][y] = *reinterpret_cast<const u32x4*>(img + q * PLANE2 + koff[s] + y * (HX * 16));
      };
      auto mma = [&](auto QA, auto QB) {
        constexpr int qa = decltype(QA)::value, qb = decltype(QB)::value;
        if constexpr (!STK) {
#pragma unroll
          for (int y = 0; y < TY; ++y)
#pragma unroll
            for (int mt = 0; mt < MT; ++mt)
              acc[y][mt] = __builtin_amdgcn_mfma_f32_16x16x32_bf16(__builtin_bit_cast(bf16x8, wa[qa][mt]),
                                                                   __builtin_bit_cast(bf16x8, xb[qb][y]), acc[y][mt], 0, 0, 0);
        }
      };
      auto mmt = [&](auto TL, auto QB) {
        constexpr int tl = decltype(TL)::value, qb = decltype(QB)::value;
        if constexpr (STK) {
#pragma unroll
          for (int y = 0; y < TY; ++y)
            acc[y][tl] = __builtin_amdgcn_mfma_f32_16x16x32_bf16(__builtin_bit_cast(bf16x8, wa[0][tl]),
                                                                 __builtin_bit_cast(bf16x8, xb[qb][y]), acc[y][tl], 0, 0, 0);
        }
      };
      xload(0, 2);
      xload(0, 1);
      xload(0, 0);
      sfor<0, NSTEP>([&](auto S) {
        constexpr int s = decltype(S)::value;
        constexpr bool last = s + 1 == NSTEP;
        const u32x4* wn = last ? wf_next : wf;
        constexpr int sn = last ? 0 : s + 1;
        constexpr int ci = s - 1;
        constexpr bool cv = ci >= 0 && ci < NL;
        if constexpr (STK) {
          __builtin_amdgcn_sched_barrier(0);
          mmt(I0{}, I2{});
          mmt(I3{}, I2{});
          __builtin_amdgcn_sched_barrier(0);
          if constexpr (!last) xload(sn, 2);
          if constexpr (cv) conv_a(ci);
          __builtin_amdgcn_sched_barrier(0);
          mmt(I0{}, I1{});
          mmt(I3{}, I1{});
          __builtin_amdgcn_sched_barrier(0);
          if constexpr (cv) conv_b(ci);
          __builtin_amdgcn_sched_barrier(0);
          mmt(I0{}, I0{});
          __builtin_amdgcn_sched_barrier(0);
          wload_t(wn, sn, 0);
          if constexpr (cv) conv_c(ci, nimg);
          __builtin_amdgcn_sched_barrier(0);
          mmt(I3{}, I0{});
          __builtin_amdgcn_sched_barrier(0);
          wload_t(wn, sn, 3);
          if constexpr (s == 2) load_pieces(P4{}, P6{});
          __builtin_amdgcn_sched_barrier(0);
          mmt(I1{}, I1{});
          __builtin_amdgcn_sched_barrier(0);
          if constexpr (!last) xload(sn, 1);
          __builtin_amdgcn_sched_barrier(0);
          mmt(I1{}, I0{});
          __builtin_amdgcn_sched_barrier(0);
          wload_t(wn, sn, 1);
          __builtin_amdgcn_sched_barrier(0);
          mmt(I2{}, I0{});
          mmt(I4{}, I0{});
          __builtin_amdgcn_sched_barrier(0);
          wload_t(wn, sn, 2);
          wload_t(wn, sn, 4);
          if constexpr (!last) xload(sn, 0);
        } else {
          __builtin_amdgcn_sched_barrier(0);
          mma(I0{}, I2{});
          __builtin_amdgcn_sched_barrier(0);
          if constexpr (!last) xload(sn, 2);
          if constexpr (cv) conv_a(ci);
          __builtin_amdgcn_sched_barrier(0);
          mma(I0{}, I1{});
          __builtin_amdgcn_sched_barrier(0);
          if constexpr (cv) conv_b(ci);
          __builtin_amdgcn_sched_barrier(0);
          mma(I0{}, I0{});
          __builtin_amdgcn_sched_barrier(0);
          wload(wn, sn, 0);
          if constexpr (cv) conv_c(ci, nimg);
          __builtin_amdgcn_sched_barrier(0);
          mma(I1{}, I0{});
          __builtin_amdgcn_sched_barrier(0);
          if constexpr (s == 2) load_pieces(P4{}, P6{});
          __builtin_amdgcn_sched_barrier(0);
          mma(I1{}, I1{});
          __builtin_amdgcn_sched_barrier(0);
          wload(wn, sn, 1);
          if constexpr (!last) xload(sn, 1);
          __builtin_amdgcn_sched_barrier(0);
          mma(I2{}, I0{});
          __builtin_amdgcn_sched_barrier(0);
          wload(wn, sn, 2);
          if constexpr (!last) xload(sn, 0);
        }
      });
      __builtin_amdgcn_sched_barrier(0);
      T2(4);
      buf ^= 1;
    }
    int z0, y0, x0;
    tile_decode(t, tiles0, a.tiles1, a.tiles2, z0, y0, x0);
    if constexpr (KS == 2) {
      __syncthreads();
      f32x4* xch = reinterpret_cast<f32x4*>(ldsh + (buf ^ 1) * BUF2) + tid;
#pragma unroll
      for (int y = 0; y < TYE; ++y)
#pragma unroll
        for (int mt = 0; mt < MT; ++mt) xch[(y * MT + mt) * 256] = half ? acc[y][mt] : acc[y + TYE][mt];
      __syncthreads();
      const f32x4* rcv = reinterpret_cast<const f32x4*>(lds + (half ^ 1) * (2 * BUF2) + (buf ^ 1) * BUF2) + tid;
#pragma unroll
      for (int y = 0; y < TYE; ++y)
#pragma unroll
        for (int mt = 0; mt < MT; ++mt) {
          const f32x4 mine = half ? acc[y + TYE][mt] : acc[y][mt];
          const f32x4 theirs = rcv[(y * MT + mt) * 256];
          acc[y][mt] = half ? theirs + mine : mine + theirs;
        }
    }
    const int gz = z0 + wave, gx = x0 + xv;
    const bool zx_ok = gz < D0 && gx < D2;
    const int yh = y0 + half * TYE;
    const uint32_t row0 = (uint32_t)((gz * D1 + yh) * D2 + gx) * (uint32_t)(Cout * 4);
    uint32_t yok = 0;
#pragma unroll
    for (int y = 0; y < TYE; ++y) yok |= (zx_ok && (yh + y) < D1) ? (1u << y) : 0u;
    T2(5);
#pragma unroll
    for (int j = 0; j < EA && j < NITEM; ++j) epi0(j, row0, yok);
#pragma unroll
    for (int j = 0; j < NITEM; ++j) {
      if (j + EA < NITEM) epi0(j + EA, row0, yok);
      epi1(j);
      epi2(j);
    }
    T2(6);
  }
  if constexpr (ST) {
    __syncthreads();
    float* red = reinterpret_cast<float*>(lds);
    const int wv = (int)threadIdx.x >> 6;
#pragma unroll
    for (int mt = 0; mt < MT; ++mt)
#pragma unroll
      for (int i = 0; i < 4; ++i) {
        float x1 = s1[mt][i], x2 = s2[mt][i];
#pragma unroll
        for (int o = 8; o > 0; o >>= 1) {
          x1 += __shfl_xor(x1, o, 64);
          x2 += __shfl_xor(x2, o, 64);
        }
        if (m == 0) {
          red[(wv * 2 + 0) * (MT * 16) + mt * 16 + 4 * g + i] = x1;
          red[(wv * 2 + 1) * (MT * 16) + mt * 16 + 4 * g + i] = x2;
        }
      }
    __syncthreads();
    float* dst = a.stats_partial + (int64_t)blockIdx.x * (2 * Cout);
    for (int e = threadIdx.x; e < MT * 16; e += 256 * KS) {
      const int c = chunk * MT * 16 + e;
      if (c < Cout) {
        float t1 = 0.f, t2 = 0.f;
#pragma unroll
        for (int w = 0; w < 4 * KS; ++w) {
          t1 += red[(2 * w) * (MT * 16) + e];
          t2 += red[(2 * w + 1) * (MT * 16) + e];
        }
        dst[c] = t1;
        dst[Cout + c] = t2;
      }
    }
  }
}

template <int MT>
struct F3Cfg {
  static constexpr int NWP = 3 * NSTEP27 * MT * 64;
  static constexpr int NWL = (NWP + 511) / 512;
  static constexpr int WBYTES = NWP * 16;
  static constexpr bool WDB = 2 * BUF + 2 * WBYTES + MT * 64 <= 160 * 1024;
  static constexpr int SMEM = 2 * BUF + (WDB ? 2 : 1) * WBYTES + MT * 64;
};

template <int MT, bool ST, int EPI0>
__global__ __launch_bounds__(512, 1) void conv3d_split_fwd3_kernel(const SplitFwdArgs a) {
  constexpr int EPI = epi_base(EPI0);
  constexpr bool RELU = EPI0 >= 5;
  using C = F3Cfg<MT>;
  constexpr int NSTEP = NSTEP27, RW = 2, NTHR = 512;
  constexpr int NITEM = RW * MT;
  constexpr bool WDB = C::WDB;
  static_assert(!ST || EPI <= 1, "statistics belong to plain forward convs");
  static_assert(NITEM <= NSTEP, "one epilogue item per K step");
  extern __shared__ __attribute__((aligned(16))) unsigned char lds[];
  unsigned char* const wlds = lds + 2 * BUF;
  float* const lbias = reinterpret_cast<float*>(wlds + (WDB ? 2 : 1) * C::WBYTES);
  const int tid = threadIdx.x, lane = tid & 63, wave = tid >> 6;
  const int m = lane & 15, g = lane >> 4, zw = wave & 3, yh = wave >> 2;
  const int chunk = blockIdx.y, nchunks = gridDim.y;
  const TileWalk walk = tile_walk(a.ntiles);
  const int tiles0 = a.ntiles / (a.tiles1 * a.tiles2);
  const int D0 = a.D0, D1 = a.D1, D2 = a.D2, Cin = a.Cin, Cout = a.Cout, ncc = a.ncc;

  int koff[NSTEP];
#pragma unroll
  for (int s = 0; s < NSTEP; ++s) {
    int tap = syn_split_tap(4 * s + g);
    if (tap < 0) tap = syn_split_tap((4 * s + g) ^ 1);
    koff[s] = ((tap / 9 * HY + (tap / 3) % 3) * HX + tap % 3) * 16;
  }
  const int xv = syn_split_voxel(m);
  const int lbase = ((zw * HY + RW * yh) * HX + xv) * 16;

  constexpr int NP = HVOX * 2, NL = 3;
  static_assert(NL * NTHR >= NP && (NL - 1) * NTHR < NP, "three staging pieces per thread");
  int prel[NL], plds[NL];
  uint32_t pmask[NL];
#pragma unroll
  for (int i = 0; i < NL; ++i) {
    int j = tid + NTHR * i;
    if (j >= NP) j -= NTHR;
    const int v = j >> 1, h = j & 1;
    const int hz = v / (HY * HX), r = v - hz * (HY * HX), hy = r / HX, hx = r - hy * HX;
    prel[i] = ((hz * D1 + hy) * D2 + hx) * Cin * 4 + h * 16;
    plds[i] = v * 16 + h * 8;
    pmask[i] = (1u << hz) | (1u << (6 + hy)) | (1u << (12 + hx));
  }
  const __amdgpu_buffer_rsrc_t rin =
      __builtin_amdgcn_make_buffer_rsrc(const_cast<float*>(a.in), 0, (int)((int64_t)D0 * D1 * D2 * Cin * 4), 0x00020000);
  f32x4 hst[NL], hnx[NL];
  auto halo_issue = [&](int t, int cc) {
    const bool none = t >= walk.end;
    int z0, y0, x0;
    tile_decode(none ? walk.pos : t, tiles0, a.tiles1, a.tiles2, z0, y0, x0);
    uint32_t bad = none ? 0xFFFFFFFFu : 0x80000000u;
    bad |= syn_oob_bits(z0 - 1, HZ, D0) | (syn_oob_bits(y0 - 1, HY, D1) << 6) | (syn_oob_bits(x0 - 1, HX, D2) << 12);
    const int base = ((((z0 - 1) * D1 + (y0 - 1)) * D2 + (x0 - 1)) * Cin + cc * 8) * 4;
#pragma unroll
    for (int i = 0; i < NL; ++i) {
      const uint32_t vo = (pmask[i] & bad) ? OOB : (uint32_t)(prel[i] + base);
      hnx[i] = __builtin_bit_cast(f32x4, __builtin_amdgcn_raw_buffer_load_b128(rin, (int)vo, 0, 0));
    }
  };
  typedef unsigned int u32x2 __attribute__((ext_vector_type(2)));
  uint32_t cp[6];
  auto conv_a = [&](int i) { syn_split3(hst[i][0], hst[i][1], cp[0], cp[1], cp[2]); };
  auto conv_b = [&](int i) { syn_split3(hst[i][2], hst[i][3], cp[3], cp[4], cp[5]); };
  auto conv_c = [&](int i, unsigned char* dst) {
    *reinterpret_cast<u32x2*>(dst + plds[i]) = (u32x2){cp[0], cp[3]};
    *reinterpret_cast<u32x2*>(dst + PLANE + plds[i]) = (u32x2){cp[1], cp[4]};
    *reinterpret_cast<u32x2*>(dst + 2 * PLANE + plds[i]) = (u32x2){cp[2], cp[5]};
  };

  const int piece_stride = nchunks * ncc * NSTEP * MT * 64;
  const __amdgpu_buffer_rsrc_t rw = __builtin_amdgcn_make_buffer_rsrc(
      const_cast<u32x4*>(a.wp), 0, (int)((int64_t)3 * piece_stride * 16), 0x00020000);
  int wsrc[C::NWL];
#pragma unroll
  for (int k = 0; k < C::NWL; ++k) {
    int j = tid + NTHR * k;
    if (j >= C::NWP) j = tid;
    const int q = j / (NSTEP * MT * 64), r = j - q * (NSTEP * MT * 64);
    wsrc[k] = (q * piece_stride + chunk * ncc * NSTEP * MT * 64 + r) * 16;
  }
  u32x4 wst[C::NWL];
  auto w_issue = [&](int cc) {
#pragma unroll
    for (int k = 0; k < C::NWL; ++k) wst[k] = __builtin_amdgcn_raw_buffer_load_b128(rw, wsrc[k] + cc * (NSTEP * MT * 64 * 16), 0, 0);
  };
  auto w_store = [&](unsigned char* dst) {
#pragma unroll
    for (int k = 0; k < C::NWL; ++k) {
      const int j = (tid + NTHR * k) >= C::NWP ? tid : tid + NTHR * k;
      *reinterpret_cast<u32x4*>(dst + j * 16) = wst[k];
    }
// ... 261 lines not shown
  const int xv = syn_split_voxel(m);
  const int par = pg * NPAR + q, pz = (par >> 2) & 1, py = (par >> 1) & 1, px = par & 1;
  const int zw0 = part * NH;
  const int lbase = ((zw0 * HY) * HX + xv) * 16 + ((pz * HY + py) * HX + px) * 16;

  constexpr int NP = HVOX * 2, NL = (NP + NTHR - 1) / NTHR;
  int prel[NL], plds[NL];
  uint32_t pmask[NL];
#pragma unroll
  for (int i = 0; i < NL; ++i) {
    const int j = tid + NTHR * i;
    const int v = j >> 1, h = j & 1;
    const int hz = v / (HY * HX), r = v - hz * (HY * HX), hy = r / HX, hx = r - hy * HX;
    prel[i] = ((hz * D1 + hy) * D2 + hx) * Cin * 4 + h * 16;
    plds[i] = v * 16 + h * 8;
    pmask[i] = j < NP ? ((1u << hz) | (1u << (6 + hy)) | (1u << (12 + hx))) : 0xFFFFFFFFu;
  }
  const __amdgpu_buffer_rsrc_t rin =
      __builtin_amdgcn_make_buffer_rsrc(const_cast<float*>(a.in), 0, (int)((int64_t)D0 * D1 * D2 * Cin * 4), 0x00020000);
  f32x4 stg[NL];
  auto load_halo = [&](int t, int cc) {
    int z0, y0, x0;
    tile_decode(t, tiles0, a.tiles1, a.tiles2, z0, y0, x0);
    uint32_t bad = 0x80000000u;
    bad |= syn_oob_bits(z0 - 1, HZ, D0) | (syn_oob_bits(y0 - 1, HY, D1) << 6) | (syn_oob_bits(x0 - 1, HX, D2) << 12);
    const int base = ((((z0 - 1) * D1 + (y0 - 1)) * D2 + (x0 - 1)) * Cin + cc * 8) * 4;
#pragma unroll
    for (int i = 0; i < NL; ++i) {
      const uint32_t vo = (pmask[i] & bad) ? OOB : (uint32_t)(prel[i] + base);
      stg[i] = __builtin_bit_cast(f32x4, __builtin_amdgcn_raw_buffer_load_b128(rin, (int)vo, 0, 0));
    }
  };
  auto store_halo = [&](int buf) {
    typedef unsigned int u32x2 __attribute__((ext_vector_type(2)));
    unsigned char* dst = lds + buf * BUF;
#pragma unroll
    for (int i = 0; i < NL; ++i) {
      if (i == NL - 1 && tid + NTHR * i >= NP) continue;
      uint32_t p0, p1, p2, q0, q1, q2;
      syn_split3(stg[i][0], stg[i][1], p0, p1, p2);
      syn_split3(stg[i][2], stg[i][3], q0, q1, q2);
      *reinterpret_cast<u32x2*>(dst + plds[i]) = (u32x2){p0, q0};
      *reinterpret_cast<u32x2*>(dst + PLANE + plds[i]) = (u32x2){p1, q1};
      *reinterpret_cast<u32x2*>(dst + 2 * PLANE + plds[i]) = (u32x2){p2, q2};
    }
  };

  const int64_t piece_stride = (int64_t)ncc * 2 * MT * 64, par_stride = 3 * piece_stride;
  const u32x4* __restrict__ wbase = a.wp + (int64_t)par * par_stride + lane;
  u32x4 wa[2][3][MT], xb[3][4];
  auto wload = [&](int cc, int s, int slot) {
#pragma unroll
    for (int pc = 0; pc < 3; ++pc)
#pragma unroll
      for (int mt = 0; mt < MT; ++mt) wa[slot][pc][mt] = wbase[pc * piece_stride + ((cc * 2 + s) * MT + mt) * 64];
  };

  const int64_t out_bytes = (int64_t)8 * D0 * D1 * D2 * Cout * 4;
  const __amdgpu_buffer_rsrc_t rout = __builtin_amdgcn_make_buffer_rsrc(a.out, 0, (int)out_bytes, 0x00020000);
  const __amdgpu_buffer_rsrc_t radd = __builtin_amdgcn_make_buffer_rsrc(
      const_cast<float*>(a.addend ? a.addend : a.out), 0, (int)out_bytes, 0x00020000);

  int buf = 0;
  if (walk.pos < walk.end) {
    load_halo(walk.pos, 0);
    store_halo(0);
    wload(0, 0, 0);
  }
  for (int t = walk.pos; t < walk.end; t += walk.stride) {
    f32x4 acc[NR][MT];
#pragma unroll
    for (int y = 0; y < NR; ++y)
#pragma unroll
      for (int mt = 0; mt < MT; ++mt) acc[y][mt] = (f32x4){0.f, 0.f, 0.f, 0.f};
    for (int cc = 0; cc < ncc; ++cc) {
      __syncthreads();
      const bool more = cc + 1 < ncc || t + walk.stride < walk.end;
      if (cc + 1 < ncc) load_halo(t, cc + 1);
      else if (t + walk.stride < walk.end) load_halo(t + walk.stride, 0);
      const unsigned char* img = lds + buf * BUF + lbase;
      const int cc_next = cc + 1 < ncc ? cc + 1 : 0;
      sfor<0, 2>([&](auto S) {
        constexpr int s = decltype(S)::value, slot = s;
        sfor<0, NH>([&](auto H) {
          constexpr int h = decltype(H)::value;
          __builtin_amdgcn_sched_barrier(0);
#pragma unroll
          for (int pc = 0; pc < 3; ++pc)
#pragma unroll
            for (int y = 0; y < 4; ++y)
              xb[pc][y] = *reinterpret_cast<const u32x4*>(img + pc * PLANE + koff[s] + (h * HY + y) * (HX * 16));
          if constexpr (h == 0) {
            if constexpr (s == 0) wload(cc, 1, 1);
            else wload(cc_next, 0, 0);
          }
          __builtin_amdgcn_sched_barrier(0);
          sfor<0, NPROD>([&](auto CC) {
            constexpr int c = decltype(CC)::value;
            constexpr int qa = split_combo_a(c, NPROD), qb = split_combo_b(c, NPROD);
#pragma unroll
            for (int y = 0; y < 4; ++y)
#pragma unroll
              for (int mt = 0; mt < MT; ++mt)
                acc[4 * h + y][mt] = __builtin_amdgcn_mfma_f32_16x16x32_bf16(
                    __builtin_bit_cast(bf16x8, wa[slot][qa][mt]), __builtin_bit_cast(bf16x8, xb[qb][y]), acc[4 * h + y][mt], 0, 0, 0);
          });
        });
      });
      __builtin_amdgcn_sched_barrier(0);
      if (more) store_halo(buf ^ 1);
      buf ^= 1;
    }
    int z0, y0, x0;
    tile_decode(t, tiles0, a.tiles1, a.tiles2, z0, y0, x0);
    const int gx = x0 + xv;
#pragma unroll
    for (int mt = 0; mt < MT; ++mt) {
      const int co = mt * 16 + 4 * g;
      f32x4 bias = {0.f, 0.f, 0.f, 0.f};
      if (a.bias && co < Cout) bias = *reinterpret_cast<const f32x4*>(a.bias + co);
#pragma unroll
      for (int r = 0; r < NR; ++r) {
        const int gz = z0 + zw0 + (r >> 2), gy = y0 + (r & 3);
        const bool vok = gz < D0 && gx < D2 && gy < D1 && co < Cout;
        const uint32_t off = vok ? (uint32_t)(((2 * gz + pz) * (2 * D1) + (2 * gy + py)) * (2 * D2) + (2 * gx + px)) *
                                       (uint32_t)(Cout * 4) + (uint32_t)(co * 4)
                                 : OOB;
        f32x4 v;
#pragma unroll
        for (int i = 0; i < 4; ++i) v[i] = acc[r][mt][i] + bias[i];
        if (a.addend) {
          const f32x4 b = __builtin_bit_cast(f32x4, __builtin_amdgcn_raw_buffer_load_b128(radd, (int)off, 0, 0));
#pragma unroll
          for (int i = 0; i < 4; ++i) v[i] += b[i];
        }
        if (a.act == 1) {
#pragma unroll
          for (int i = 0; i < 4; ++i) v[i] = act_f<RELU>(v[i]);
        }
        __builtin_amdgcn_raw_buffer_store_b128(__builtin_bit_cast(u32x4, v), rout, (int)off, 0, 0);
      }
    }
  }
}

inline int split_upfwd_grid_x(int ntiles, int ngroups) { return syn_tile_grid_x(256 / ngroups, ntiles); }
inline int split_grid_x(int ntiles, int nchunks) { return syn_tile_grid_x(512 / nchunks, ntiles); }
inline int split_wgrad_grid_x(int ntiles, int gy) {
  int gx = std::max(1, 256 / gy);
  if (gx > ntiles) gx = ntiles;
  return gx;
}

inline int split_tiles1(const int s[3]) { return (s[1] + TY - 1) / TY; }
inline int split_tiles2(const int s[3]) { return (s[2] + TX - 1) / TX; }
inline int split_ntiles(const int s[3]) { return ((s[0] + TZ - 1) / TZ) * split_tiles1(s) * split_tiles2(s); }

inline SplitFwdArgs split_fwd_args(const float* in, const float* wp, const float* bias, const float* addend, float* out,
                                   float* stats_partial, const int s[3], int Cin, int Cout, int act, int stacked) {
  SplitFwdArgs a;
  a.in = in;
  a.wp = reinterpret_cast<const u32x4*>(wp);
  a.bias = bias;
  a.addend = addend;
  a.out = out;
  a.stats_partial = stats_partial;
  a.D0 = s[0]; a.D1 = s[1]; a.D2 = s[2];
  a.Cin = Cin; a.Cout = Cout; a.ncc = Cin / 8;
  a.tiles1 = split_tiles1(s);
  a.tiles2 = split_tiles2(s);
  a.ntiles = split_ntiles(s);
  a.act = act;
  a.stacked = stacked;
  return a;
}

template <class F>
int with_mt(int mt, F&& f) {
  if (mt == 1) return f(std::integral_constant<int, 1>{});
  if (mt == 2) return f(std::integral_constant<int, 2>{});
  return f(std::integral_constant<int, 3>{});
}
inline int split_epi(const SplitFwdArgs& a) {
  if (a.act == 3) return a.addend ? 7 : 5;
  if (a.act == 4) return 6;
  return a.act + ((a.addend && a.act < 2) ? 3 : 0);
}
template <bool ST, class F>
int with_epi(int epi, F&& f) {
  if constexpr (ST) {
    if (epi == 5) return f(std::integral_constant<int, 5>{});
    return epi == 1 ? f(std::integral_constant<int, 1>{}) : f(std::integral_constant<int, 0>{});
  } else {
    switch (epi) {
      case 0: return f(std::integral_constant<int, 0>{});
      case 1: return f(std::integral_constant<int, 1>{});
      case 2: return f(std::integral_constant<int, 2>{});
      case 3: return f(std::integral_constant<int, 3>{});
      case 5: return f(std::integral_constant<int, 5>{});
      case 6: return f(std::integral_constant<int, 6>{});
      case 7: return f(std::integral_constant<int, 7>{});
      default: return f(std::integral_constant<int, 4>{});
    }
  }
}

inline bool relu_args(const SplitFwdArgs& a, SplitFwdArgs& b) {
  b = a;
  if (a.act < 3) return false;
  b.act -= 2;
  return true;
}

template <int MT, int NPAR>
int launch_split_upfwd(const SplitFwdArgs& a0, int nprod, hipStream_t st) {
  constexpr int NG = 8 / NPAR;
  constexpr auto k9r = conv3d_split_upfwd_kernel<MT, NPAR, 9, true>, k9 = conv3d_split_upfwd_kernel<MT, NPAR, 9>;
  constexpr auto k6r = conv3d_split_upfwd_kernel<MT, NPAR, 6, true>, k6 = conv3d_split_upfwd_kernel<MT, NPAR, 6>;
  SplitFwdArgs a;
  const bool relu = relu_args(a0, a);
  const dim3 grid(split_upfwd_grid_x(a.ntiles, NG), 1, NG);
  if (nprod == 9) launch_smem<k9, k9r>(relu, grid, dim3(512), 2 * BUF, st, a);
  else launch_smem<k6, k6r>(relu, grid, dim3(512), 2 * BUF, st, a);
  SYN_CHECK_LAUNCH();
  return SYNTHSR_OK;
}

enum class FwdRoute { generic, fwd2, fwd2_halves, fwd3, refuse };
inline FwdRoute split_fwd_route(int ntiles, int nchunks, int ncc, int mt, int Cout, int stacked, int upm, int nprod) {
  if (stacked) return (upm == 0 && mt == 2 && nprod == 6) ? FwdRoute::fwd2 : FwdRoute::refuse;
  if (upm != 0 || nprod != 6) return FwdRoute::generic;
  const int64_t units = (int64_t)ntiles * nchunks;
  if (!syn_split_replanned(ntiles, (Cout + 15) / 16, mt) && nchunks >= 2 && units >= 512 && units < 1024) return FwdRoute::fwd3;
  const bool halves = (int64_t)split_grid_x(ntiles, nchunks) * nchunks <= 256 && ncc >= 4 && (ncc % 2) == 0;
  return halves ? FwdRoute::fwd2_halves : FwdRoute::fwd2;
}
inline int split_fwd_grid_x(FwdRoute route, int ntiles, int nchunks) {
  return route == FwdRoute::fwd3 ? split_upfwd_grid_x(ntiles, nchunks) : split_grid_x(ntiles, nchunks);
}

template <auto Kern>
int launch_split_fwd_k(const SplitFwdArgs& a, dim3 grid, int threads, size_t smem, hipStream_t st) {
  max_dyn_smem<Kern>(smem);
  hipLaunchKernelGGL(Kern, grid, dim3(threads), smem, st, a);
  SYN_CHECK_LAUNCH();
  return SYNTHSR_OK;
}

template <int MT, bool ST, int UPM>
int launch_split_fwd(const SplitFwdArgs& a0, FwdRoute route, int nchunks, int nprod, hipStream_t st) {
  if (route == FwdRoute::refuse) return SYNTHSR_EINVAL;
  const dim3 grid(split_fwd_grid_x(route, a0.ntiles, nchunks), nchunks);
  if constexpr (UPM == 0) {
    const int epi = split_epi(a0);
    if (a0.stacked) {
      if constexpr (MT == 2)
        return with_epi<ST>(epi, [&](auto E) {
          return launch_split_fwd_k<conv3d_split_fwd2_kernel<2, ST, decltype(E)::value, true>>(a0, grid, 256, 2 * BUF2 + 2 * 16 * 4, st);
        });
      return SYNTHSR_EINVAL;
    }
    if (route == FwdRoute::fwd3)
      return with_epi<ST>(epi, [&](auto E) {
        return launch_split_fwd_k<conv3d_split_fwd3_kernel<MT, ST, decltype(E)::value>>(a0, grid, 512, F3Cfg<MT>::SMEM, st);
      });
    if (route != FwdRoute::generic)
      return with_epi<ST>(epi, [&](auto E) {
        constexpr int EPI = decltype(E)::value;
        if (route == FwdRoute::fwd2_halves)
          return launch_split_fwd_k<conv3d_split_fwd2_kernel<MT, ST, EPI, false, 2>>(a0, grid, 512, 4 * BUF2 + MT * 16 * 4, st);
        return launch_split_fwd_k<conv3d_split_fwd2_kernel<MT, ST, EPI, false>>(a0, grid, 256, 2 * BUF2 + MT * 16 * 4, st);
      });
  }
  constexpr auto k9r = conv3d_split_fwd_kernel<MT, ST, UPM, 9, true>, k9 = conv3d_split_fwd_kernel<MT, ST, UPM, 9>;
  constexpr auto k6r = conv3d_split_fwd_kernel<MT, ST, UPM, 6, true>, k6 = conv3d_split_fwd_kernel<MT, ST, UPM, 6>;
  SplitFwdArgs a;
  const bool relu = relu_args(a0, a);
  if (nprod == 9) launch_smem<k9, k9r>(relu, grid, dim3(256), 2 * BUF, st, a);
  else launch_smem<k6, k6r>(relu, grid, dim3(256), 2 * BUF, st, a);
  SYN_CHECK_LAUNCH();
  return SYNTHSR_OK;
}

typedef short s16x4 __attribute__((ext_vector_type(4)));
typedef __attribute__((address_space(3))) s16x4 lds_s16x4;
__device__ __forceinline__ u32x4 tr_read8(const unsigned char* p_lo, const unsigned char* p_hi) {
  const s16x4 lo = __builtin_amdgcn_ds_read_tr16_b64_v4i16((lds_s16x4*)p_lo);
  const s16x4 hi = __builtin_amdgcn_ds_read_tr16_b64_v4i16((lds_s16x4*)p_hi);
  return __builtin_bit_cast(u32x4, __builtin_shufflevector(lo, hi, 0, 1, 2, 3, 4, 5, 6, 7));
}

struct SplitWgArgs {
  const float* in;
  const float* dout;
  float* dw;
  float* dbias;
  int D0, D1, D2, Cin, Cout, cin_total, ci_off, ncc, nco, tiles1, tiles2, ntiles, ciw;
  int64_t det_stride;
};

template <int COW, int CIW = 8>
struct WgCfg {
  static constexpr int NT = (COW + 15) / 16, DROWB = COW * 2, DPLANE = TZ * TY * TX * DROWB;
  static constexpr int XB = CIW * 2, XPLANE = HVOX * XB;
  static constexpr int NRT = CIW == 24 ? 44 : 14 * (CIW / 8);
  static constexpr int RT = CIW == 24 ? 11 : (COW <= 24 ? 14 : 7);
  static constexpr int BUFB = 3 * XPLANE + 3 * DPLANE + 64;
  static constexpr bool DBUF = 2 * BUFB <= 160 * 1024;
  static constexpr int NBUF = DBUF ? 2 : 1;
};

template <int COW, int NPROD = 6, bool STK = false, int CIW = 8>
__global__ __launch_bounds__(512, 1) void conv3d_split_wgrad_kernel(const SplitWgArgs a) {
  constexpr bool PL = CIW == 24, BAL = CIW == 24;
  constexpr int QP = HVOX * 8;
  static_assert(!STK || (COW == 24 && NPROD == 6), "stacked column tiles: 24 columns, six products");
  static_assert(CIW == 8 || (CIW == 16 && COW == 48) || (CIW == 24 && COW == 24 && STK),
                "16 input channels per workgroup: the 48-column kernel; 24: the stacked 24-column kernel");
  using C = WgCfg<COW, CIW>;
  constexpr int NT = C::NT, DROWB = C::DROWB, DPLANE = C::DPLANE, RT = C::RT, NW = 8, NTHR = 512;
  constexpr int XB = C::XB, WG_XPLANE = C::XPLANE, XQ = CIW / 4;
  constexpr int NXP = HVOX * XQ, NXL = (NXP + NTHR - 1) / NTHR;
  constexpr int DQ = COW / 4, NDP = TZ * TY * TX * DQ, NDL = NDP / NTHR;
  static_assert(NDP % NTHR == 0, "dz pieces divide among the threads");
  extern __shared__ __attribute__((aligned(16))) unsigned char lds[];
  const int tid = threadIdx.x, lane = tid & 63, wave = tid >> 6;
  const int g = lane >> 4, li = lane & 15, lrow = li >> 2, lq = li & 3;
  constexpr int GROUPS = C::NRT / RT, WPG = NW / GROUPS, KPW = 8 / WPG;
  const int rh = CIW == 24 ? __builtin_amdgcn_readfirstlane(wave / WPG) : wave / WPG, wg = wave % WPG;
  const int rt0 = BAL ? rh * (RT - 1) + (rh > 0 ? 1 : 0) : rh * RT;
  const bool slot10 = !BAL || rh == 0 || rh == GROUPS - 1;
  const int cc = blockIdx.y % a.ncc, oc = blockIdx.y / a.ncc;
  const TileWalk walk = tile_walk(a.ntiles);
  const int tiles0 = a.ntiles / (a.tiles1 * a.tiles2);
  const int D0 = a.D0, D1 = a.D1, D2 = a.D2, Cin = a.Cin, Cout = a.Cout;

  int aoff[RT];
#pragma unroll
  for (int q = 0; q < RT; ++q) {
    const int Q = 4 * (rt0 + q) + lq;
    int tap = CIW == 8 ? 2 * (rh * RT + q) + (lq >> 1) : (CIW == 16 ? rh * RT + q : Q / 6);
    if (tap > 26) tap = 26;
    const int tvox = (tap / 9 * HY + (tap / 3) % 3) * HX + tap % 3;
    if constexpr (PL) aoff[q] = tvox * 8 + (Q % 6) * QP;
    else aoff[q] = tvox * XB + (CIW == 8 ? (lq & 1) : (CIW == 16 ? lq : Q % 6)) * 8;
  }
  const int ks0 = wg * KPW, kz = ks0 >> 1, kyb = 2 * (ks0 & 1);
  constexpr int XVB = PL ? 8 : XB;
  auto akoff = [](int kj) { return (uint32_t)(((kj >> 1) * HY * HX + (kj & 1) * 2 * HX) * XVB); };
  auto bkoff = [](int kj) { return (uint32_t)(((kj >> 1) * TY * TX + (kj & 1) * 2 * TX) * DROWB); };
  static_assert(KPW == 1 || KPW == 2 || KPW == 4, "K steps of a wave: whole x-row pairs of consecutive z planes");
  const int vx = 4 * (g & 1) + lrow, vr = g >> 1;
  const uint32_t abase = (uint32_t)((((kz * HY + kyb + vr) * HX) + vx) * XVB);
  const uint32_t bbase = (uint32_t)(3 * WG_XPLANE) + (uint32_t)((((kz * TY + kyb + vr) * TX) + vx) * DROWB + lq * 8);
  constexpr uint32_t ZOFF = (uint32_t)(3 * WG_XPLANE + 3 * DPLANE);
  const uint32_t bvox = bbase - (uint32_t)(lq * 8);
  const uint32_t u3off = bvox + (uint32_t)((lq >> 1) * DPLANE + 32 + (lq & 1) * 8);
  const uint32_t u4off = lq < 2 ? bvox + (uint32_t)(2 * DPLANE + 32 + (lq & 1) * 8) : ZOFF;
  const uint32_t u4hi = lq < 2 ? (uint32_t)(8 * DROWB) : 0u;
  auto u4koff = [&](int kj) { return lq < 2 ? bkoff(kj) : 0u; };
  if constexpr (STK) {
    if (tid < 2 * C::NBUF) *reinterpret_cast<uint64_t*>(lds + (tid >> 1) * C::BUFB + ZOFF + (tid & 1) * 8) = 0ull;
  }

  static_assert(XB == XQ * 8 && DROWB == DQ * 8, "pieces tile the voxel rows");
  constexpr bool XPLN = CIW == 16;
  static_assert(!XPLN || (NXL == HZ && NTHR / XQ >= HY * HX), "one halo plane per staging piece");
  int xrel[XPLN ? 1 : NXL];
  uint32_t xmask[XPLN ? 1 : NXL];
  const int xq = tid & 3, xr = tid >> 2;
  const int xps = D1 * D2 * Cin * 4;
  if constexpr (XPLN) {
    const int hy = xr / HX, hx = xr - hy * HX;
    xrel[0] = (hy * D2 + hx) * Cin * 4 + xq * 16;
    xmask[0] = xr < HY * HX ? ((1u << (6 + hy)) | (1u << (12 + hx))) : 0xFFFFFFFFu;
  } else {
#pragma unroll
    for (int i = 0; i < NXL; ++i) {
      const int j = tid + NTHR * i;
      const int v = j / XQ, h = j % XQ;
      const int hz = v / (HY * HX), r = v - hz * (HY * HX), hy = r / HX, hx = r - hy * HX;
      xrel[i] = ((hz * D1 + hy) * D2 + hx) * Cin * 4 + h * 16;
      xmask[i] = j < NXP ? ((1u << hz) | (1u << (6 + hy)) | (1u << (12 + hx))) : 0xFFFFFFFFu;
    }
  }
  constexpr bool DPLN = XPLN && COW == 48;
  int drel[DPLN ? 1 : NDL];
  uint32_t dmask[DPLN ? 1 : NDL];
  const int dps = 2 * D1 * D2 * Cout * 4;
  if constexpr (DPLN) {
    static_assert(!DPLN || NDL == 6, "two plane pairs x three quad groups");
    const int vz = xr / (TY * TX), vy = (xr / TX) % TY, vxx = xr % TX;
    dmask[0] = (1u << vz) | (1u << (4 + vy)) | (1u << (8 + vxx));
    drel[0] = ((vz * D1 + vy) * D2 + vxx) * Cout * 4 + (oc * COW + xq * 4) * 4;
  } else {
#pragma unroll
    for (int i = 0; i < NDL; ++i) {
      const int j = tid + NTHR * i;
      const int v = j / DQ, c4 = j - v * DQ;
      const int vz = v / (TY * TX), vy = (v / TX) % TY, vxx = v % TX;
      const int co = oc * COW + c4 * 4;
      dmask[i] = co < Cout ? ((1u << vz) | (1u << (4 + vy)) | (1u << (8 + vxx))) : 0xFFFFFFFFu;
      drel[i] = ((vz * D1 + vy) * D2 + vxx) * Cout * 4 + co * 4;
    }
  }
  const __amdgpu_buffer_rsrc_t rin =
      __builtin_amdgcn_make_buffer_rsrc(const_cast<float*>(a.in), 0, (int)((int64_t)D0 * D1 * D2 * Cin * 4), 0x00020000);
  const __amdgpu_buffer_rsrc_t rdo =
      __builtin_amdgcn_make_buffer_rsrc(const_cast<float*>(a.dout), 0, (int)((int64_t)D0 * D1 * D2 * Cout * 4), 0x00020000);
  f32x4 xst[NXL], dst[NDL];
  auto load_tile = [&](int t) {
    int z0, y0, x0;
    tile_decode(t, tiles0, a.tiles1, a.tiles2, z0, y0, x0);
    uint32_t bad = 0x80000000u;
    bad |= syn_oob_bits(z0 - 1, HZ, D0) | (syn_oob_bits(y0 - 1, HY, D1) << 6) | (syn_oob_bits(x0 - 1, HX, D2) << 12);
    const int base = ((((z0 - 1) * D1 + (y0 - 1)) * D2 + (x0 - 1)) * Cin + cc * CIW) * 4;
    int xps_t = xps;
    uint32_t xm_t = xmask[0];
    if constexpr (XPLN) {
      asm volatile("" : "+s"(xps_t));
      asm volatile("" : "+v"(xm_t));
    }
#pragma unroll
    for (int i = 0; i < NXL; ++i) {
// ... 356 lines not shown
  T2(0);
  int cz = 0, cy = 0, cx = 0, nz = 0, ny = 0, nx = 0;
  if (walk.pos < walk.end) {
    tile_decode(walk.pos, tiles0, a.tiles1, a.tiles2, cz, cy, cx);
    load_x(cz, cy, cx);
    load_dz(cz, cy, cx, 0, 0);
    load_dz(cz, cy, cx, 1, 1);
    store_x();
#pragma unroll
    for (int k = 0; k < NDL; ++k) store_dz1(0, k, 0);
  }
  __syncthreads();
  T2(1);
  for (int t = walk.pos; t < walk.end; t += walk.stride) {
    const bool more = t + walk.stride < walk.end;
    if (more) tile_decode(t + walk.stride, tiles0, a.tiles1, a.tiles2, nz, ny, nx);
    sfor<0, UW_NST>([&](auto ST) {
      constexpr int st = decltype(ST)::value, zp = st >> 1, kj = st & 1;
      T2(2);
      T3(0);
      if constexpr (st + 2 < UW_NST) {
        load_dz(cz, cy, cx, st + 2, kj);
      } else {
        if (more) load_dz(nz, ny, nx, st + 2 - UW_NST, kj);
      }
      if constexpr (st == UW_NST - 1) {
        if (more) load_x(nz, ny, nx);
      }
      const bool next = st + 1 < UW_NST || more;
      {
        constexpr uint32_t ak = (uint32_t)((zp * HY * HX + kj * 2 * HX) * UW_XB), bk = (uint32_t)(kj * UW_DBUF);
        u32x4 bfr[3][2], afr[2][3];
#pragma unroll
        for (int p = 0; p < 3; ++p)
          bfr[p][0] = tr_read8(lds + bbase + bk + p * UW_DPLANE, lds + bbase + bk + p * UW_DPLANE + 8 * UW_DROWB);
        bfr[0][1] = tr_read8(lds + u3off + bk, lds + u3off + bk + 8 * UW_DROWB);
        bfr[1][1] = tr_read8(lds + u4off + (lq < 2 ? bk : 0u), lds + u4off + (lq < 2 ? bk : 0u) + u4hi);
        auto aload = [&](int q, int slot) {
#pragma unroll
          for (int p = 0; p < 3; ++p)
            afr[slot][p] = tr_read8(lds + aaddr[q] + ak + p * UW_XPLANE, lds + aaddr[q] + ak + p * UW_XPLANE + 8 * UW_XB);
        };
        aload(0, 0);
        sfor<0, RT>([&](auto Q) {
          constexpr int q = decltype(Q)::value;
          __builtin_amdgcn_sched_barrier(0);
          if constexpr (q + 1 < RT) aload(q + 1, (q + 1) & 1);
          __builtin_amdgcn_sched_barrier(0);
          auto mm = [&](int xa, int pb, int nb, int ac) {
            acc[q][ac] = __builtin_amdgcn_mfma_f32_16x16x32_bf16(__builtin_bit_cast(bf16x8, afr[q & 1][xa]),
                                                                  __builtin_bit_cast(bf16x8, bfr[pb][nb]), acc[q][ac], 0, 0, 0);
          };
          mm(0, 2, 0, 0);
          mm(0, 1, 1, 1);
          mm(2, 0, 0, 0);
          mm(2, 0, 1, 1);
          mm(1, 1, 0, 0);
          mm(1, 0, 1, 1);
          mm(0, 1, 0, 0);
          mm(0, 0, 1, 1);
          mm(1, 0, 0, 0);
          mm(0, 0, 0, 0);
          if constexpr (q >= 2 && (q & 1) == 0) {
            if (next) store_dz1(kj ^ 1, q / 2 - 1, kj ^ 1);
          }
        });
        __builtin_amdgcn_sched_barrier(0);
      }
      T2(3);
      T3(1);
      T2(4);
#ifdef SYN_SPLIT_TIMING
      ++n3;
#endif
      if constexpr (st == UW_NST - 1) {
        __syncthreads();
        if (more) store_x();
      }
      __syncthreads();
      T2(5);
    });
    cz = nz; cy = ny; cx = nx;
  }
#pragma unroll
  for (int q = 0; q < RT; ++q)
#pragma unroll
    for (int i = 0; i < 4; ++i) acc[q][1][i] += __shfl_down(acc[q][1][i], 8, 16);
  float* dwp = a.dwc + (size_t)blockIdx.x * a.det_stride + (size_t)par * 27 * Cin * Cout;
#pragma unroll
  for (int q = 0; q < RT; ++q) {
    const int slot = ((pz + (q >> 2)) * 3 + py + ((q >> 1) & 1)) * 3 + px + (q & 1);
#pragma unroll
    for (int n = 0; n < 2; ++n) {
      const int col = n * 16 + li;
      if (col >= 24) continue;
#pragma unroll
      for (int i = 0; i < 4; ++i) {
        const int ci = cc * 16 + 4 * g + i;
        atomicAdd(dwp + ((int64_t)slot * Cin + ci) * Cout + oc * 24 + col, acc[q][n][i]);
      }
    }
  }
}

}

extern "C" __attribute__((visibility("hidden"))) int syn_split_upwgrad(const float* lo, const float* dout, float* dwc,
                                                                        const int s[3], int Cin, int Cout, int nprod,
                                                                        hipStream_t st) {
  if (nprod != 6 || (Cin % 16) != 0 || (Cout % 24) != 0) return SYNTHSR_EINVAL;
  const int64_t vox = (int64_t)s[0] * s[1] * s[2];
  if (vox * Cin * 4 >= (1ll << 31) || 8 * vox * Cout * 4 >= (1ll << 31)) return SYNTHSR_EINVAL;
  SplitUpWgArgs a;
  a.lo = lo;
  a.dout = dout;
  a.dwc = dwc;
  a.D0 = s[0]; a.D1 = s[1]; a.D2 = s[2];
  a.Cin = Cin; a.Cout = Cout;
  a.ncc = Cin / 16;
  a.nco = Cout / 24;
  a.tiles1 = split_tiles1(s);
  a.tiles2 = split_tiles2(s);
  a.ntiles = split_ntiles(s);
  const int gy = a.ncc * a.nco;
  const int gx = split_wgrad_grid_x(a.ntiles, gy);
  max_dyn_smem<conv3d_split_upwgrad_kernel>(UW_LDS);
  DetRun det;
  float* no_dbias = nullptr;
  if (const int rc_ = syn_det_prepare(&det, &a.dwc, &no_dbias, (int64_t)8 * 27 * Cin * Cout, Cout, gx, st)) return rc_;
  a.det_stride = det.stride;
  hipLaunchKernelGGL(conv3d_split_upwgrad_kernel, dim3(gx, gy), dim3(512), (size_t)UW_LDS, st, a);
  SYN_CHECK_LAUNCH();
  return syn_det_finish(&det, st);
}

extern "C" int synthsr_split_tile_schedule(int kernel, int ntiles, int ny, int block_x, int block_yz, int out[4]) {
  if (ntiles < 1 || ny < 1 || block_x < 0 || block_yz < 0 || !out) return SYNTHSR_EINVAL;
  int gx;
  if (kernel == 0) gx = split_grid_x(ntiles, ny);
  else if (kernel == 1) gx = split_wgrad_grid_x(ntiles, ny);
  else if (kernel == 2) gx = split_upfwd_grid_x(ntiles, ny);
  else return SYNTHSR_EINVAL;
  out[0] = gx;
  if (block_x >= gx) return SYNTHSR_EINVAL;
  const TileWalk w = tile_walk_of(gx, block_x, gx * block_yz, ntiles);
  out[1] = w.pos;
  out[2] = w.end;
  out[3] = w.stride;
  return SYNTHSR_OK;
}

extern "C" __attribute__((visibility("hidden"))) int syn_split_fwd_halves(const int s[3], int Cin, int nchunks, int stacked,
                                                                           int nprod) {
  return split_fwd_route(split_ntiles(s), nchunks, Cin / 8, 3, 0, stacked, 0, nprod) == FwdRoute::fwd2_halves ? 1 : 0;
}

extern "C" __attribute__((visibility("hidden"))) int syn_split_fwd(const float* in, const float* wp, const float* bias,
                                                                    const float* addend, float* out, const int s[3], int Cin,
                                                                    int Cout, int mt, int nchunks, int act, float* stats,
                                                                    float* partial, int upm, int stacked, int nprod,
                                                                    hipStream_t st) {
  if (nprod != 6 && nprod != 9) return SYNTHSR_EINVAL;
  if ((Cin % 8) != 0 || (Cout % 4) != 0 || mt < 1 || mt > 3 || nchunks < 1 || (upm != 0 && upm != 2)) return SYNTHSR_EINVAL;
  if (stacked && (Cout != 24 || mt != 2 || nchunks != 1 || upm != 0 || nprod != 6)) return SYNTHSR_EINVAL;
  if (act < 0 || act > 4 || (stats && (!partial || addend || act == 2 || act == 4 || upm))) return SYNTHSR_EINVAL;
  if (upm && (bias || addend || act != 0)) return SYNTHSR_EINVAL;
  const int64_t vox = (int64_t)s[0] * s[1] * s[2];
  if ((upm ? 8 : 1) * vox * Cin * 4 >= (1ll << 31) || vox * Cout * 4 >= (1ll << 31)) return SYNTHSR_EINVAL;
  const SplitFwdArgs a = split_fwd_args(in, wp, bias, addend, out, stats ? partial : nullptr, s, Cin, Cout, act, stacked);
  const FwdRoute route = split_fwd_route(a.ntiles, nchunks, a.ncc, mt, Cout, stacked, upm, nprod);
  if (stats) {
    const int rc = with_mt(mt, [&](auto M) { return launch_split_fwd<decltype(M)::value, true, 0>(a, route, nchunks, nprod, st); });
    if (rc != SYNTHSR_OK) return rc;
    return synthsr_bn_stats_from_partials(partial, split_fwd_grid_x(route, a.ntiles, nchunks), vox, Cout, stats, (synthsr_stream_t)st);
  }
  if (upm == 2) return with_mt(mt, [&](auto M) { return launch_split_fwd<decltype(M)::value, false, 2>(a, route, nchunks, nprod, st); });
  return with_mt(mt, [&](auto M) { return launch_split_fwd<decltype(M)::value, false, 0>(a, route, nchunks, nprod, st); });
}

extern "C" __attribute__((visibility("hidden"))) int syn_split_upfwd(const float* lo, const float* wp, const float* bias,
                                                                      const float* addend, float* out, const int s[3], int Cin,
                                                                      int Cout, int mt, int act, int nprod, hipStream_t st) {
  if (nprod != 6 && nprod != 9) return SYNTHSR_EINVAL;
  if ((Cin % 8) != 0 || (Cout % 4) != 0 || mt < 1 || mt > 3 || Cout > 16 * mt || (act != 0 && act != 1 && act != 3)) return SYNTHSR_EINVAL;
  const int64_t vox = (int64_t)s[0] * s[1] * s[2];
  if (vox * Cin * 4 >= (1ll << 31) || 8 * vox * Cout * 4 >= (1ll << 31)) return SYNTHSR_EINVAL;
  const SplitFwdArgs a = split_fwd_args(lo, wp, bias, addend, out, nullptr, s, Cin, Cout, act, 0);
  if (mt == 1) return launch_split_upfwd<1, 4>(a, nprod, st);
  if (mt == 2) return launch_split_upfwd<2, 4>(a, nprod, st);
  return launch_split_upfwd<3, 2>(a, nprod, st);
}

extern "C" __attribute__((visibility("hidden"))) int syn_split_wgrad(const float* in, const float* dout, float* dw, float* dbias,
                                                                      const int s[3], int cin_total, int ci_off, int Cin,
                                                                      int Cout, int nprod, hipStream_t st) {
  if (nprod != 6 && nprod != 9) return SYNTHSR_EINVAL;
  if ((Cin % 8) != 0 || (Cout % 24) != 0) return SYNTHSR_EINVAL;
  const int64_t vox = (int64_t)s[0] * s[1] * s[2];
  if (vox * Cin * 4 >= (1ll << 31) || vox * Cout * 4 >= (1ll << 31)) return SYNTHSR_EINVAL;
  SplitWgArgs a;
  a.in = in;
  a.dout = dout;
  a.dw = dw;
  a.dbias = dbias;
  a.D0 = s[0]; a.D1 = s[1]; a.D2 = s[2];
  a.Cin = Cin; a.Cout = Cout; a.cin_total = cin_total; a.ci_off = ci_off;
  const bool c48 = (Cout % 48) == 0;
  a.ciw = (c48 && (Cin % 16) == 0 && nprod == 6) ? 16 : 8;
  if (!c48 && Cin == 24 && nprod == 6) a.ciw = 24;
  a.ncc = Cin / a.ciw;
  a.nco = c48 ? Cout / 48 : Cout / 24;
  a.tiles1 = split_tiles1(s);
  a.tiles2 = split_tiles2(s);
  a.ntiles = split_ntiles(s);
  a.det_stride = 0;
  return c48 ? launch_split_wgrad<48>(a, nprod, st) : launch_split_wgrad<24>(a, nprod, st);
}
```

Measured before the change: 53.44 volumes/s.

## Add 4x8x8 tile geometry to split forward conv when it yields fewer tiles

Templates the split forward conv kernel on tile geometry, adding a 4x8x8 voxel tile alongside the existing 4x4x16 one. The 8x8 geometry is picked automatically when it needs fewer tiles for the volume shape. At 160^3 this applies to the 40^3 and 20^3 levels, where 16-wide x tiles waste padding. It also shrinks the halo image to five staging pieces per thread. The cost is more kernel instantiations and new per-lane voxel/row mapping code that has to stay correct, including the out-of-bounds mask shifts.

```diff
diff --git a/include/synthsr_hip_tuning.h b/include/synthsr_hip_tuning.h
--- a/include/synthsr_hip_tuning.h
+++ b/include/synthsr_hip_tuning.h
@@ -5,6 +5,12 @@
 #endif
 
 int synthsr_split_tile_schedule(int kernel, int ntiles, int ny, int block_x, int block_yz, int out[4]);
+
+int synthsr_split_tile_geometry(const int shape[3]);
+int synthsr_split_tile_origin(int geo, const int shape[3], int p, int out[6]);
+int synthsr_split_fwd_geo(const float* in, const float* wpacked, const float* bias, const float* addend, float* out,
+                          const int shape[3], int Cin, int Cout, int mt, int nchunks, int act, float* stats, float* partial,
+                          int geo, void* stream);
 
 int synthsr_set_deterministic(int on);
 int synthsr_set_deterministic_workspace(void* planes, unsigned long long bytes);
diff --git a/synthsr_amd/_lib.py b/synthsr_amd/_lib.py
--- a/synthsr_amd/_lib.py
+++ b/synthsr_amd/_lib.py
@@ -52,6 +52,9 @@
     'synthsr_bn_stats_from_partials': (c_int, [_P, c_int, c_int64, c_int, _P, _S]),
     'synthsr_conv3d_fwd_add': (c_int, [_C, _P, _P, _P, _P, _P, POINTER(c_int), c_int, c_int, c_int, _S]),
     'synthsr_split_tile_schedule': (c_int, [c_int, c_int, c_int, c_int, c_int, POINTER(c_int)]),
+    'synthsr_split_tile_geometry': (c_int, [POINTER(c_int)]),
+    'synthsr_split_tile_origin': (c_int, [c_int, POINTER(c_int), c_int, POINTER(c_int)]),
+    'synthsr_split_fwd_geo': (c_int, [_P, _P, _P, _P, _P, POINTER(c_int), c_int, c_int, c_int, c_int, c_int, _P, _P, c_int, _S]),
     'synthsr_conv3d_wgrad_runs_split': (c_int, [_C, POINTER(c_int), c_int, c_int]),
     'synthsr_set_deterministic': (c_int, [c_int]),
     'synthsr_set_deterministic_workspace': (c_int, [_P, c_uint64]),
diff --git a/synthsr_amd/csrc/common.h b/synthsr_amd/csrc/common.h
--- a/synthsr_amd/csrc/common.h
+++ b/synthsr_amd/csrc/common.h
@@ -263,17 +263,22 @@
   else return elu_dy(y);
 }
 
-constexpr int TZ = 4, TY = 4, TX = 16, HZ = TZ + 2, HY = TY + 2, HX = TX + 2, HVOX = HZ * HY * HX;
+template <int GEO>
+struct TileGeo {
+  static constexpr int TY = GEO ? 8 : 4, TX = GEO ? 8 : 16, HY = TY + 2, HX = TX + 2, HVOX = 6 * HY * HX;
+};
+constexpr int TZ = 4, TY = TileGeo<0>::TY, TX = TileGeo<0>::TX, HZ = TZ + 2, HY = TY + 2, HX = TX + 2, HVOX = HZ * HY * HX;
 constexpr int SLAB_Z = 4;
-__device__ __forceinline__ void tile_decode(int p, int tiles0, int tiles1, int tiles2, int& z0, int& y0, int& x0) {
+template <int TY_ = TY, int TX_ = TX>
+__host__ __device__ __forceinline__ void tile_decode(int p, int tiles0, int tiles1, int tiles2, int& z0, int& y0, int& x0) {
   const int t12 = tiles1 * tiles2;
   const int s = p / (SLAB_Z * t12), r = p - s * SLAB_Z * t12;
-  const int sz = min(SLAB_Z, tiles0 - s * SLAB_Z);
+  const int sz = tiles0 - s * SLAB_Z < SLAB_Z ? tiles0 - s * SLAB_Z : SLAB_Z;
   const int t1 = r / (sz * tiles2), rr = r - t1 * sz * tiles2;
   const int zz = rr / tiles2, t2 = rr - zz * tiles2;
   z0 = (s * SLAB_Z + zz) * TZ;
-  y0 = t1 * TY;
-  x0 = t2 * TX;
+  y0 = t1 * TY_;
+  x0 = t2 * TX_;
 }
 #endif
 static inline int syn_tile_grid_x(int slots, int ntiles) {
@@ -284,6 +289,13 @@
   return gx;
 }
 
+static inline int syn_split_tiles1(const int s[3], int geo) { return geo ? (s[1] + 7) / 8 : (s[1] + 3) / 4; }
+static inline int syn_split_tiles2(const int s[3], int geo) { return geo ? (s[2] + 7) / 8 : (s[2] + 15) / 16; }
+static inline int syn_split_ntiles(const int s[3], int geo) {
+  return ((s[0] + 3) / 4) * syn_split_tiles1(s, geo) * syn_split_tiles2(s, geo);
+}
+static inline int syn_split_tile_geo(const int s[3]) { return syn_split_ntiles(s, 1) < syn_split_ntiles(s, 0) ? 1 : 0; }
+
 __host__ __device__ inline bool syn_split_replanned(int vox_tiles, int co_tiles, int mt) {
   if (mt != 2 || co_tiles <= 3 || (co_tiles % 3) != 0 || (co_tiles % 2) != 0) return false;
   const long long u3 = (long long)vox_tiles * (co_tiles / 3);
@@ -306,6 +318,8 @@
   return 4 * (p & 1) + 2 * h + (p >> 1);
 }
 __host__ __device__ constexpr int syn_split_voxel(int m) { return m < 4 ? 2 * m : (m >= 12 ? 2 * m - 16 : 2 * m - 7); }
+__host__ __device__ constexpr int syn_split_voxel88(int m) { return m < 4 ? 2 * m : (m >= 12 ? 2 * m - 24 : (m < 8 ? 2 * m - 7 : 2 * m - 15)); }
+__host__ __device__ constexpr int syn_split_row88(int m) { return m >= 8 ? 1 : 0; }
 
 __device__ static inline float syn_wave_sum(float v) {
 #pragma unroll
diff --git a/synthsr_amd/csrc/conv3d.hip b/synthsr_amd/csrc/conv3d.hip
--- a/synthsr_amd/csrc/conv3d.hip
+++ b/synthsr_amd/csrc/conv3d.hip
@@ -2638,7 +2638,7 @@
 extern "C" int syn_split_fwd_halves(const int s[3], int Cin, int nchunks, int stacked, int nprod);
 extern "C" int syn_split_fwd(const float* in, const float* wp, const float* bias, const float* addend, float* out,
                              const int s[3], int Cin, int Cout, int mt, int nchunks, int act, float* stats, float* partial,
-                             int upm, int stacked, int nprod, hipStream_t st);
+                             int upm, int stacked, int nprod, int geo, hipStream_t st);
 
 inline bool wgrad_takes_split(const int s[3], int Cin, int Cout) {
   const int64_t vox = (int64_t)s[0] * s[1] * s[2];
@@ -3462,7 +3462,7 @@
   const FwdPlan pl = plan_fwd(shape, Cin, Cout);
   if (pl.split)
     return syn_split_fwd(in, wpacked, bias, nullptr, out, shape, Cin, Cout, pl.mt, pl.nchunks, act, nullptr, nullptr, 0,
-                         pl.stacked, cfg().nprod, (hipStream_t)stream);
+                         pl.stacked, cfg().nprod, -1, (hipStream_t)stream);
   return dispatch_fwd_ck(pl, in, wpacked, bias, out, shape, Cin, Cout, act, stream, ConvExt{0, nullptr, 0});
 }
 
@@ -3477,7 +3477,7 @@
   const FwdPlan pl = plan_fwd(shape, Cin, Cout);
   if (pl.split)
     return syn_split_fwd(in, wpacked, bias, addend, out, shape, Cin, Cout, pl.mt, pl.nchunks, act, nullptr, nullptr, 0,
-                         pl.stacked, cfg().nprod, (hipStream_t)stream);
+                         pl.stacked, cfg().nprod, -1, (hipStream_t)stream);
   return dispatch_fwd_ck(pl, in, wpacked, bias, out, shape, Cin, Cout, act, stream, ConvExt{0, addend, 0});
 }
 
@@ -3493,7 +3493,7 @@
     float* partial = ctx_scratch((size_t)512 * 2 * Cout * sizeof(float));
     if (!partial) return SYNTHSR_EWORKSPACE;
     return syn_split_fwd(in, wpacked, bias, nullptr, out, shape, Cin, Cout, pl.mt, pl.nchunks, act, stats, partial, 0,
-                         pl.stacked, cfg().nprod, (hipStream_t)stream);
+                         pl.stacked, cfg().nprod, -1, (hipStream_t)stream);
   }
   if (pl.p4 && nvox * Cin * 4 < (1ll << 31))
     return launch_fwd_p4(in, wpacked, bias, out, shape, Cin, pl, act, (hipStream_t)stream, nullptr, stats);
@@ -3522,7 +3522,7 @@
   const FwdPlan pl = plan_fwd(lo_shape, Cout, Cl, 0);
   if (pl.split)
     return syn_split_fwd(dout, wpacked8, nullptr, nullptr, dlo, lo_shape, Cout, Cl, pl.mt, pl.nchunks, 0, nullptr, nullptr, 2, 0,
-                         cfg().nprod, (hipStream_t)stream);
+                         cfg().nprod, -1, (hipStream_t)stream);
   return dispatch_fwd_ck(pl, dout, wpacked8, nullptr, dlo, lo_shape, Cout, Cl, 0, stream, ConvExt{2, nullptr, pl.count()});
 }
 
diff --git a/synthsr_amd/csrc/conv_split.hip b/synthsr_amd/csrc/conv_split.hip
--- a/synthsr_amd/csrc/conv_split.hip
+++ b/synthsr_amd/csrc/conv_split.hip
@@ -407,18 +407,28 @@
   }
 }
 
-constexpr int PLANE2 = 6 * 256 * 8;
-constexpr int BUF2 = 3 * PLANE2;
-static_assert(PLANE2 >= PLANE, "padded plane holds the halo image");
+template <int GEO>
+struct F2Cfg {
+  static constexpr int NL = (TileGeo<GEO>::HVOX * 2 + 255) / 256;
+  static constexpr int PLANE2 = NL * 256 * 8;
+  static constexpr int BUF2 = 3 * PLANE2;
+};
+static_assert(F2Cfg<0>::PLANE2 >= PLANE && F2Cfg<0>::NL == 6 && F2Cfg<1>::NL == 5, "padded plane holds the halo image");
 constexpr int STK_TILES = 5;
 
 constexpr int epi_base(int epi) { return epi == 5 ? 1 : (epi == 6 ? 2 : (epi == 7 ? 4 : epi)); }
 
-template <int MT, bool ST, int EPI0, bool STK, int KS = 1>
+
+template <int MT, bool ST, int EPI0, bool STK, int KS = 1, int GEO = 0>
 __global__ __launch_bounds__(256 * KS, KS == 1 ? 2 : 1) void conv3d_split_fwd2_kernel(const SplitFwdArgs a) {
   static_assert(KS == 1 || (KS == 2 && !STK), "split-K halves: the plain layout");
+  static_assert(GEO == 0 || !STK, "4x8x8 tiles: the plain layout");
+  using G = TileGeo<GEO>;
+  constexpr int HY = G::HY, HX = G::HX, HVOX = G::HVOX;
+  constexpr int PLANE2 = F2Cfg<GEO>::PLANE2, BUF2 = F2Cfg<GEO>::BUF2;
   constexpr int NSTEP = NSTEP27;
-  constexpr int TYE = TY / KS;
+  constexpr int NR = 4;
+  constexpr int TYE = NR / KS;
   constexpr int NITEM = TYE * MT;
   constexpr int NWT = STK ? STK_TILES : MT;
   constexpr int EPI = epi_base(EPI0);
@@ -442,11 +452,12 @@
     if (tap < 0) tap = syn_split_tap((4 * s + g) ^ 1);
     koff[s] = ((tap / 9 * HY + (tap / 3) % 3) * HX + tap % 3) * 16;
   }
-  const int xv = syn_split_voxel(m);
-  const int lbase = (wave * HY * HX + xv) * 16;
-
-  constexpr int NP = HVOX * 2, NL = 6;
-  static_assert(NL * 256 >= NP, "six staging pieces per thread cover the halo image");
+  const int xv = GEO ? syn_split_voxel88(m) : syn_split_voxel(m);
+  const int yv = GEO ? 4 * syn_split_row88(m) : 0;
+  const int lbase = ((wave * HY + yv) * HX + xv) * 16;
+
+  constexpr int NP = HVOX * 2, NL = F2Cfg<GEO>::NL;
+  static_assert(NL * 256 >= NP && NL >= 5 && NL <= 6, "staging pieces per thread cover the halo image; steps 1 .. NL convert them");
   int prel[NL];
   uint32_t pmask[NL];
 #pragma unroll
@@ -455,7 +466,7 @@
     const int v = j >> 1, h = j & 1;
     const int hz = v / (HY * HX), r = v - hz * (HY * HX), hy = r / HX, hx = r - hy * HX;
     prel[i] = ((hz * D1 + hy) * D2 + hx) * Cin * 4 + h * 16;
-    pmask[i] = j < NP ? ((1u << hz) | (1u << (6 + hy)) | (1u << (12 + hx))) : 0xFFFFFFFFu;
+    pmask[i] = j < NP ? ((1u << hz) | (1u << (6 + hy)) | (1u << (6 + HY + hx))) : 0xFFFFFFFFu;
   }
   const int plds0 = (tid >> 1) * 16 + (tid & 1) * 8;
   const __amdgpu_buffer_rsrc_t rin =
@@ -468,9 +479,9 @@
   auto halo_where = [&](int t, int cc, bool none) {
     if (t != hw_tile) {
       int z0, y0, x0;
-      tile_decode(t, tiles0, a.tiles1, a.tiles2, z0, y0, x0);
+      tile_decode<G::TY, G::TX>(t, tiles0, a.tiles1, a.tiles2, z0, y0, x0);
       uint32_t bad = 0x80000000u;
-      bad |= syn_oob_bits(z0 - 1, HZ, D0) | (syn_oob_bits(y0 - 1, HY, D1) << 6) | (syn_oob_bits(x0 - 1, HX, D2) << 12);
+      bad |= syn_oob_bits(z0 - 1, HZ, D0) | (syn_oob_bits(y0 - 1, HY, D1) << 6) | (syn_oob_bits(x0 - 1, HX, D2) << (6 + HY));
       hw_bad = bad;
       hw_base0 = (((z0 - 1) * D1 + (y0 - 1)) * D2 + (x0 - 1)) * Cin * 4;
       hw_tile = t;
@@ -488,7 +499,7 @@
   };
   using P0 = std::integral_constant<int, 0>;
   using P4 = std::integral_constant<int, 4>;
-  using P6 = std::integral_constant<int, 6>;
+  using PL = std::integral_constant<int, NL>;
   typedef unsigned int u32x2 __attribute__((ext_vector_type(2)));
   uint32_t cp[6];
   auto conv_a = [&](int i) { syn_split3(stg[i][0], stg[i][1], cp[0], cp[1], cp[2]); };
@@ -521,7 +532,7 @@
     lbias[tid] = (a.bias && co < Cout) ? a.bias[co] : 0.f;
   }
 
-  u32x4 wa[STK ? 1 : 3][STK ? STK_TILES : MT], xb[3][TY];
+  u32x4 wa[STK ? 1 : 3][STK ? STK_TILES : MT], xb[3][NR];
   auto wload = [&](const u32x4* wf, int s, int q) {
     if constexpr (!STK) {
 #pragma unroll
@@ -537,7 +548,7 @@
   using I3 = std::integral_constant<int, 3>;
   using I4 = std::integral_constant<int, 4>;
 
-  f32x4 acc[TY][NWT];
+  f32x4 acc[NR][NWT];
   constexpr int EA = EPI >= 2 ? 3 : 1, ENB = EA + 1;
   f32x4 ev, eb[ENB];
   uint32_t eoff[ENB];
@@ -599,7 +610,7 @@
   T2(0);
   if (walk.pos < walk.end) {
     halo_where(walk.pos, half, false);
-    load_pieces(P0{}, P6{});
+    load_pieces(P0{}, PL{});
 #pragma unroll
     for (int i = 0; i < NL; ++i) {
       conv_a(i);
@@ -618,7 +629,7 @@
   T2(1);
   for (int t = walk.pos; t < walk.end; t += walk.stride) {
 #pragma unroll
-    for (int y = 0; y < TY; ++y)
+    for (int y = 0; y < NR; ++y)
 #pragma unroll
       for (int tl = 0; tl < NWT; ++tl) acc[y][tl] = (f32x4){0.f, 0.f, 0.f, 0.f};
     for (int cc = half; cc < ncc; cc += KS) {
@@ -635,13 +646,13 @@
       unsigned char* nimg = ldsh + (buf ^ 1) * BUF2;
       auto xload = [&](int s, int q) {
 #pragma unroll
-        for (int y = 0; y < TY; ++y) xb[q][y] = *reinterpret_cast<const u32x4*>(img + q * PLANE2 + koff[s] + y * (HX * 16));
+        for (int y = 0; y < NR; ++y) xb[q][y] = *reinterpret_cast<const u32x4*>(img + q * PLANE2 + koff[s] + y * (HX * 16));
       };
       auto mma = [&](auto QA, auto QB) {
         constexpr int qa = decltype(QA)::value, qb = decltype(QB)::value;
         if constexpr (!STK) {
 #pragma unroll
-          for (int y = 0; y < TY; ++y)
+          for (int y = 0; y < NR; ++y)
 #pragma unroll
             for (int mt = 0; mt < MT; ++mt)
               acc[y][mt] = __builtin_amdgcn_mfma_f32_16x16x32_bf16(__builtin_bit_cast(bf16x8, wa[qa][mt]),
@@ -652,7 +663,7 @@
         constexpr int tl = decltype(TL)::value, qb = decltype(QB)::value;
         if constexpr (STK) {
 #pragma unroll
-          for (int y = 0; y < TY; ++y)
+          for (int y = 0; y < NR; ++y)
             acc[y][tl] = __builtin_amdgcn_mfma_f32_16x16x32_bf16(__builtin_bit_cast(bf16x8, wa[0][tl]),
                                                                  __builtin_bit_cast(bf16x8, xb[qb][y]), acc[y][tl], 0, 0, 0);
         }
@@ -688,7 +699,7 @@
           mmt(I3{}, I0{});
           __builtin_amdgcn_sched_barrier(0);
           wload_t(wn, sn, 3);
-          if constexpr (s == 2) load_pieces(P4{}, P6{});
+          if constexpr (s == 2) load_pieces(P4{}, PL{});
           __builtin_amdgcn_sched_barrier(0);
           mmt(I1{}, I1{});
           __builtin_amdgcn_sched_barrier(0);
@@ -722,7 +733,7 @@
           __builtin_amdgcn_sched_barrier(0);
           mma(I1{}, I0{});
           __builtin_amdgcn_sched_barrier(0);
-          if constexpr (s == 2) load_pieces(P4{}, P6{});
+          if constexpr (s == 2) load_pieces(P4{}, PL{});
           __builtin_amdgcn_sched_barrier(0);
           mma(I1{}, I1{});
           __builtin_amdgcn_sched_barrier(0);
@@ -740,7 +751,7 @@
       buf ^= 1;
     }
     int z0, y0, x0;
-    tile_decode(t, tiles0, a.tiles1, a.tiles2, z0, y0, x0);
+    tile_decode<G::TY, G::TX>(t, tiles0, a.tiles1, a.tiles2, z0, y0, x0);
     if constexpr (KS == 2) {
       __syncthreads();
       f32x4* xch = reinterpret_cast<f32x4*>(ldsh + (buf ^ 1) * BUF2) + tid;
@@ -761,7 +772,8 @@
     }
     const int gz = z0 + wave, gx = x0 + xv;
     const bool zx_ok = gz < D0 && gx < D2;
-    const int yh = y0 + half * TYE;
+    static_assert(KS == 1 || TYE * MT * 256 * 16 <= BUF2, "the exchanged accumulators fit an image buffer");
+    const int yh = y0 + half * TYE + yv;
     const uint32_t row0 = (uint32_t)((gz * D1 + yh) * D2 + gx) * (uint32_t)(Cout * 4);
     uint32_t yok = 0;
 #pragma unroll
@@ -1329,12 +1341,12 @@
   return gx;
 }
 
-inline int split_tiles1(const int s[3]) { return (s[1] + TY - 1) / TY; }
-inline int split_tiles2(const int s[3]) { return (s[2] + TX - 1) / TX; }
-inline int split_ntiles(const int s[3]) { return ((s[0] + TZ - 1) / TZ) * split_tiles1(s) * split_tiles2(s); }
+inline int split_tiles1(const int s[3], int geo = 0) { return syn_split_tiles1(s, geo); }
+inline int split_tiles2(const int s[3], int geo = 0) { return syn_split_tiles2(s, geo); }
+inline int split_ntiles(const int s[3], int geo = 0) { return syn_split_ntiles(s, geo); }
 
 inline SplitFwdArgs split_fwd_args(const float* in, const float* wp, const float* bias, const float* addend, float* out,
-                                   float* stats_partial, const int s[3], int Cin, int Cout, int act, int stacked) {
+                                   float* stats_partial, const int s[3], int Cin, int Cout, int act, int stacked, int geo = 0) {
   SplitFwdArgs a;
   a.in = in;
   a.wp = reinterpret_cast<const u32x4*>(wp);
@@ -1344,9 +1356,9 @@
   a.stats_partial = stats_partial;
   a.D0 = s[0]; a.D1 = s[1]; a.D2 = s[2];
   a.Cin = Cin; a.Cout = Cout; a.ncc = Cin / 8;
-  a.tiles1 = split_tiles1(s);
-  a.tiles2 = split_tiles2(s);
-  a.ntiles = split_ntiles(s);
+  a.tiles1 = split_tiles1(s, geo);
+  a.tiles2 = split_tiles2(s, geo);
+  a.ntiles = split_ntiles(s, geo);
   a.act = act;
   a.stacked = stacked;
   return a;
@@ -1404,13 +1416,18 @@
 }
 
 enum class FwdRoute { generic, fwd2, fwd2_halves, fwd3, refuse };
-inline FwdRoute split_fwd_route(int ntiles, int nchunks, int ncc, int mt, int Cout, int stacked, int upm, int nprod) {
+inline FwdRoute split_fwd_route(int ntiles, int ntiles416, int nchunks, int ncc, int mt, int Cout, int stacked, int upm, int nprod,
+                                int geo) {
+  if (geo && (stacked || upm != 0 || nprod != 6)) return FwdRoute::refuse;
   if (stacked) return (upm == 0 && mt == 2 && nprod == 6) ? FwdRoute::fwd2 : FwdRoute::refuse;
   if (upm != 0 || nprod != 6) return FwdRoute::generic;
   const int64_t units = (int64_t)ntiles * nchunks;
-  if (!syn_split_replanned(ntiles, (Cout + 15) / 16, mt) && nchunks >= 2 && units >= 512 && units < 1024) return FwdRoute::fwd3;
-  const bool halves = (int64_t)split_grid_x(ntiles, nchunks) * nchunks <= 256 && ncc >= 4 && (ncc % 2) == 0;
+  if (!geo && !syn_split_replanned(ntiles, (Cout + 15) / 16, mt) && nchunks >= 2 && units >= 512 && units < 1024) return FwdRoute::fwd3;
+  const bool halves = (int64_t)split_grid_x(ntiles416, nchunks) * nchunks <= 256 && ncc >= 4 && (ncc % 2) == 0;
   return halves ? FwdRoute::fwd2_halves : FwdRoute::fwd2;
+}
+inline int split_fwd_geo(const int s[3], int stacked, int upm, int nprod) {
+  return (stacked || upm != 0 || nprod != 6) ? 0 : syn_split_tile_geo(s);
 }
 inline int split_fwd_grid_x(FwdRoute route, int ntiles, int nchunks) {
   return route == FwdRoute::fwd3 ? split_upfwd_grid_x(ntiles, nchunks) : split_grid_x(ntiles, nchunks);
@@ -1425,7 +1442,7 @@
 }
 
 template <int MT, bool ST, int UPM>
-int launch_split_fwd(const SplitFwdArgs& a0, FwdRoute route, int nchunks, int nprod, hipStream_t st) {
+int launch_split_fwd(const SplitFwdArgs& a0, FwdRoute route, int nchunks, int nprod, int geo, hipStream_t st) {
   if (route == FwdRoute::refuse) return SYNTHSR_EINVAL;
   const dim3 grid(split_fwd_grid_x(route, a0.ntiles, nchunks), nchunks);
   if constexpr (UPM == 0) {
@@ -1433,7 +1450,7 @@
     if (a0.stacked) {
       if constexpr (MT == 2)
         return with_epi<ST>(epi, [&](auto E) {
-          return launch_split_fwd_k<conv3d_split_fwd2_kernel<2, ST, decltype(E)::value, true>>(a0, grid, 256, 2 * BUF2 + 2 * 16 * 4, st);
+          return launch_split_fwd_k<conv3d_split_fwd2_kernel<2, ST, decltype(E)::value, true>>(a0, grid, 256, 2 * F2Cfg<0>::BUF2 + 2 * 16 * 4, st);
         });
       return SYNTHSR_EINVAL;
     }
@@ -1444,9 +1461,13 @@
     if (route != FwdRoute::generic)
       return with_epi<ST>(epi, [&](auto E) {
         constexpr int EPI = decltype(E)::value;
-        if (route == FwdRoute::fwd2_halves)
-          return launch_split_fwd_k<conv3d_split_fwd2_kernel<MT, ST, EPI, false, 2>>(a0, grid, 512, 4 * BUF2 + MT * 16 * 4, st);
-        return launch_split_fwd_k<conv3d_split_fwd2_kernel<MT, ST, EPI, false>>(a0, grid, 256, 2 * BUF2 + MT * 16 * 4, st);
+        auto go = [&](auto GE) {
+          constexpr int GEO = decltype(GE)::value, BUF2 = F2Cfg<GEO>::BUF2;
+          if (route == FwdRoute::fwd2_halves)
+            return launch_split_fwd_k<conv3d_split_fwd2_kernel<MT, ST, EPI, false, 2, GEO>>(a0, grid, 512, 4 * BUF2 + MT * 16 * 4, st);
+          return launch_split_fwd_k<conv3d_split_fwd2_kernel<MT, ST, EPI, false, 1, GEO>>(a0, grid, 256, 2 * BUF2 + MT * 16 * 4, st);
+        };
+        return geo ? go(std::integral_constant<int, 1>{}) : go(std::integral_constant<int, 0>{});
       });
   }
   constexpr auto k9r = conv3d_split_fwd_kernel<MT, ST, UPM, 9, true>, k9 = conv3d_split_fwd_kernel<MT, ST, UPM, 9>;
@@ -2109,14 +2130,18 @@
 
 extern "C" __attribute__((visibility("hidden"))) int syn_split_fwd_halves(const int s[3], int Cin, int nchunks, int stacked,
                                                                            int nprod) {
-  return split_fwd_route(split_ntiles(s), nchunks, Cin / 8, 3, 0, stacked, 0, nprod) == FwdRoute::fwd2_halves ? 1 : 0;
-}
+  const int geo = split_fwd_geo(s, stacked, 0, nprod);
+  return split_fwd_route(split_ntiles(s, geo), split_ntiles(s), nchunks, Cin / 8, 3, 0, stacked, 0, nprod, geo) == FwdRoute::fwd2_halves ? 1 : 0;
+}
+
 
 extern "C" __attribute__((visibility("hidden"))) int syn_split_fwd(const float* in, const float* wp, const float* bias,
                                                                     const float* addend, float* out, const int s[3], int Cin,
                                                                     int Cout, int mt, int nchunks, int act, float* stats,
                                                                     float* partial, int upm, int stacked, int nprod,
-                                                                    hipStream_t st) {
+                                                                    int geo, hipStream_t st) {
+  if (geo < 0) geo = split_fwd_geo(s, stacked, upm, nprod);
+  if (geo > 1) return SYNTHSR_EINVAL;
   if (nprod != 6 && nprod != 9) return SYNTHSR_EINVAL;
   if ((Cin % 8) != 0 || (Cout % 4) != 0 || mt < 1 || mt > 3 || nchunks < 1 || (upm != 0 && upm != 2)) return SYNTHSR_EINVAL;
   if (stacked && (Cout != 24 || mt != 2 || nchunks != 1 || upm != 0 || nprod != 6)) return SYNTHSR_EINVAL;
@@ -2124,15 +2149,42 @@
   if (upm && (bias || addend || act != 0)) return SYNTHSR_EINVAL;
   const int64_t vox = (int64_t)s[0] * s[1] * s[2];
   if ((upm ? 8 : 1) * vox * Cin * 4 >= (1ll << 31) || vox * Cout * 4 >= (1ll << 31)) return SYNTHSR_EINVAL;
-  const SplitFwdArgs a = split_fwd_args(in, wp, bias, addend, out, stats ? partial : nullptr, s, Cin, Cout, act, stacked);
-  const FwdRoute route = split_fwd_route(a.ntiles, nchunks, a.ncc, mt, Cout, stacked, upm, nprod);
+  const SplitFwdArgs a = split_fwd_args(in, wp, bias, addend, out, stats ? partial : nullptr, s, Cin, Cout, act, stacked, geo);
+  const FwdRoute route = split_fwd_route(a.ntiles, split_ntiles(s), nchunks, a.ncc, mt, Cout, stacked, upm, nprod, geo);
   if (stats) {
-    const int rc = with_mt(mt, [&](auto M) { return launch_split_fwd<decltype(M)::value, true, 0>(a, route, nchunks, nprod, st); });
+    const int rc = with_mt(mt, [&](auto M) { return launch_split_fwd<decltype(M)::value, true, 0>(a, route, nchunks, nprod, geo, st); });
     if (rc != SYNTHSR_OK) return rc;
     return synthsr_bn_stats_from_partials(partial, split_fwd_grid_x(route, a.ntiles, nchunks), vox, Cout, stats, (synthsr_stream_t)st);
   }
-  if (upm == 2) return with_mt(mt, [&](auto M) { return launch_split_fwd<decltype(M)::value, false, 2>(a, route, nchunks, nprod, st); });
-  return with_mt(mt, [&](auto M) { return launch_split_fwd<decltype(M)::value, false, 0>(a, route, nchunks, nprod, st); });
+  if (upm == 2) return with_mt(mt, [&](auto M) { return launch_split_fwd<decltype(M)::value, false, 2>(a, route, nchunks, nprod, geo, st); });
+  return with_mt(mt, [&](auto M) { return launch_split_fwd<decltype(M)::value, false, 0>(a, route, nchunks, nprod, geo, st); });
+}
+
+extern "C" int synthsr_split_fwd_geo(const float* in, const float* wp, const float* bias, const float* addend, float* out,
+                                     const int s[3], int Cin, int Cout, int mt, int nchunks, int act, float* stats,
+                                     float* partial, int geo, synthsr_stream_t st) {
+  if (!in || !wp || !out || !s || s[0] < 1 || s[1] < 1 || s[2] < 1 || Cin < 8 || Cout < 4 || geo < 0 || geo > 1) return SYNTHSR_EINVAL;
+  if (mt < 1 || mt > 3 || nchunks != (Cout + 16 * mt - 1) / (16 * mt)) return SYNTHSR_EINVAL;
+  if ((act == 2 || act == 4) && (!addend || addend == out)) return SYNTHSR_EINVAL;
+  return syn_split_fwd(in, wp, bias, addend, out, s, Cin, Cout, mt, nchunks, act, stats, partial, 0, 0, 6, geo, (hipStream_t)st);
+}
+
+extern "C" int synthsr_split_tile_geometry(const int s[3]) {
+  if (!s || s[0] < 1 || s[1] < 1 || s[2] < 1) return SYNTHSR_EINVAL;
+  return syn_split_tile_geo(s);
+}
+extern "C" int synthsr_split_tile_origin(int geo, const int s[3], int p, int out[6]) {
+  if (!s || !out || s[0] < 1 || s[1] < 1 || s[2] < 1 || geo < 0 || geo > 1) return SYNTHSR_EINVAL;
+  out[0] = (s[0] + TZ - 1) / TZ;
+  out[1] = split_tiles1(s, geo);
+  out[2] = split_tiles2(s, geo);
+  const int n = split_ntiles(s, geo);
+  if (p >= n) return SYNTHSR_EINVAL;
+  if (p >= 0) {
+    if (geo) tile_decode<TileGeo<1>::TY, TileGeo<1>::TX>(p, out[0], out[1], out[2], out[3], out[4], out[5]);
+    else tile_decode(p, out[0], out[1], out[2], out[3], out[4], out[5]);
+  }
+  return n;
 }
 
 extern "C" __attribute__((visibility("hidden"))) int syn_split_upfwd(const float* lo, const float* wp, const float* bias,
```

Result: no change. 53.56 volumes/s, median of 2 (+0.2%).
